# ZhangHH233/Retinal_OCT_Image_Segmentation_via_Deep_Learning

Measured on AMD Instinct MI355X. Metric: B-scans/sec (train fwd+bwd) at batch 32, 512x1024, higher is better.
Workload: dtype bf16; 1 GPU; SOTAS/Layers_Segment UNet(1,8,init_features=32) train step, 512x1024, batch 32/GPU (BASELINE configs[1]); global_batch=32, parallelism=dp1, hip_graph=False

## Files before the change

### include/oct_hip.h

```cpp
#ifndef OCT_HIP_H
#define OCT_HIP_H

#include <stddef.h>
#include <stdint.h>

#ifdef __cplusplus
extern "C" {
#endif

#define OCT_VERSION 220

#define OCT_DT_BF16 0
#define OCT_DT_F32 1

#define OCT_OK 0
#define OCT_IMG_SHIFT_ALL 2
#define OCT_E_INVALID (-22)
#define OCT_E_LAUNCH (-5)
#define OCT_E_NODEVICE (-19)

#define OCT_XF_NONE 0
#define OCT_XF_AFFINE_RELU 1
#define OCT_XF_AFFINE 2

#define OCT_IN_PLAIN 0
#define OCT_IN_S2D 1
#define OCT_OUT_PLAIN 0
#define OCT_OUT_D2S 1

#define OCT_PACK_CONV_FPROP 0
#define OCT_PACK_CONV_DGRAD 1
#define OCT_PACK_DECONV_FPROP 2
#define OCT_PACK_DECONV_DGRAD 3
#define OCT_PACK_1X1_DGRAD 4
#define OCT_PACK_1X1_FPROP 5
#define OCT_PACK_CONV3D_FPROP 6
#define OCT_PACK_CONV3D_DGRAD 7
#define OCT_PACK_DECONV3D_FPROP 8
#define OCT_PACK_DECONV3D_DGRAD 9

const char* oct_version_string(void);
int oct_version(void);
int oct_get_last_error(char* buf, size_t len);
int oct_device_count(void);

typedef struct OctConvDesc {
  int dtype;
  int n, h, w;
  int c0, c1;
  int cout;
  int taps;
  int xform0, xform1;
  int in_mode, out_mode;
  int split;
  int want_stats;
  int kh, kw;
  int depth;
  int out_img_mul, out_img_add;
} OctConvDesc;

typedef struct OctConvArgs {
  const void* x0; const void* x1;
  const float* scale0; const float* shift0;
  const float* scale1; const float* shift1;
  const void* wpacked;
  const float* bias;
  void* y0; void* y1;
  float* stat_partials;
} OctConvArgs;

int oct_conv_stat_blocks(const OctConvDesc* d);
size_t oct_packed_weight_elems(int rows, int taps, int kch);
int oct_pack_weights(int mode, int dtype, const float* w, void* wpacked, int cout, int cin, void* stream);
int oct_pack_weights_kk(int mode, int dtype, const float* w, void* wpacked, int cout, int cin, int kh, int kw,
                        void* stream);
int oct_pack_weights3d(int mode, int dtype, const float* w, void* wpacked, int cout, int cin, int kdi, void* stream);
#define OCT_PACK_BATCH_MAX 96
typedef struct OctPackJob {
  int mode, cout, cin, reserved;
  const float* w;
  void* wpacked;
} OctPackJob;
int oct_pack_weights_batch(int dtype, int count, const OctPackJob* jobs, void* stream);
int oct_conv_forward(const OctConvDesc* d, const OctConvArgs* a, void* stream);

typedef struct OctWgradDesc {
  int dtype;
  int n, h, w;
  int c0, c1;
  int cout;
  int taps;
  int xform0, xform1;
  int dy_mode;
  int kh, kw;
  int depth;
  int in_img_shift;
  int dy_img_mul, dy_img_add;
  int partials;
} OctWgradDesc;
typedef struct OctWgradArgs {
  const void* x0; const void* x1;
  const float* scale0; const float* shift0;
  const float* scale1; const float* shift1;
  const void* dy;
  float* dwp;
  float* dbias;
  const void* dy_y; const float* dy_coef; const float* dy_scale; const float* dy_shift;
  float* dbias_partials;
} OctWgradArgs;
int oct_conv_wgrad(const OctWgradDesc* d, const OctWgradArgs* a, void* stream);
int oct_conv_wgrad_partials(const OctWgradDesc* d);
int oct_reduce_bias_partials(const float* part, int nparts, int rows, int channels, float* dbias, int accumulate,
                             void* stream);
int oct_conv_wgrad_fused_apply_ok(const OctWgradDesc* d);
int oct_conv_wgrad_all_depth_taps_ok(const OctWgradDesc* d);
typedef struct OctConvBwdFusedArgs {
  const void* x;
  const float* scale; const float* shift;
  const float* mean; const float* invstd;
  const void* dy;
  const void* wpacked;
  void* dx;
  float* dwp;
  float* partials;
} OctConvBwdFusedArgs;
int oct_conv_backward_fused_ok(const OctWgradDesc* d);
int oct_conv_backward_fused_blocks(const OctWgradDesc* d);
int oct_conv_backward_fused(const OctWgradDesc* d, const OctConvBwdFusedArgs* a, void* stream);
int oct_unpack_wgrad(int mode, const float* dwp, float* grad, int cout, int cin, int accumulate, void* stream);
int oct_unpack_wgrad_kk(const float* dwp, float* grad, int cout, int cin, int kh, int kw, int accumulate, void* stream);
int oct_unpack_wgrad3d(int mode, const float* dwp, float* grad, int cout, int cin, int kdi, int accumulate, void* stream);
typedef struct OctUnpackJob {
  int mode, cout, cin, accumulate;
  int nparts, reserved;
  const float* dwp;
  float* grad;
} OctUnpackJob;
int oct_unpack_wgrad_batch(int count, const OctUnpackJob* jobs, void* stream);

int oct_bn_finalize(const float* partials, int nblocks, int c, double count,
                    const float* gamma, const float* beta, float eps, float momentum,
                    float* running_mean, float* running_var,
                    float* mean, float* invstd, float* scale, float* shift, const float* conv_bias,
                    void* stream);
int oct_bn_eval_coeffs(int c, const float* gamma, const float* beta, const float* running_mean,
                       const float* running_var, float eps, float* scale, float* shift,
                       const float* conv_bias, void* stream);

int oct_bn_relu_pool_fwd(int dtype, const void* y, const float* scale, const float* shift,
                         void* pooled, int n, int h, int w, int c, void* stream);
int oct_bn_relu_fwd(int dtype, const void* y, const float* scale, const float* shift,
                    void* out, size_t npix, int c, void* stream);

int oct_dact_bn_reduce(int dtype, const void* da, const void* dpool, const void* y,
                       const float* scale, const float* shift, const float* mean,
                       const float* invstd, void* g, float* partials, int n, int h, int w, int c,
                       void* stream);
int oct_dact_bn_reduce_blocks(int n, int h, int w, int c, int has_pool);
int oct_bn_bwd_apply_pool_ok(int dtype, int n, int h, int w, int c);
int oct_bn_bwd_apply_pool(int dtype, const void* da, const void* dpool, const void* y, const float* scale,
                          const float* shift, const float* coef, void* dy, int n, int h, int w, int c, void* stream);
int oct_bn_bwd_finalize(const float* partials, int nblocks, int c, double count,
                        const float* gamma, const float* mean, const float* invstd,
                        float* dgamma, float* dbeta, float* coef , int accumulate,
                        void* stream);
int oct_bn_bwd_apply(int dtype, void* g, const void* y, const float* coef, const float* scale,
                     const float* shift, size_t npix, int c, void* stream);
int oct_bn_bwd_apply_to(int dtype, void* dst, const void* g, const void* y, const float* coef, const float* scale,
                        const float* shift, size_t npix, int c, void* stream);
int oct_rowdot_ok(int c, int k);
int oct_rowdot_blocks(size_t npix, int c);
int oct_rowdot_fwd(int dtype, const void* x, const float* w, void* y, float* stats, size_t npix, int c, int k, void* stream);
int oct_rowdot_bwd_data(int dtype, const void* dy, const float* w, void* dx, size_t npix, int c, int k, void* stream);
int oct_rowdot_bwd_weight(int dtype, const void* dy, const void* x, float* dw, float* partials, size_t npix, int c, int k,
                          int accumulate, void* stream);
int oct_rowdot_bwd_weight_bias(int dtype, const void* dy, const void* x, float* dw, float* dbias, float* partials, size_t npix, int c,
                               int k, int accumulate, void* stream);

int oct_channel_sum(int dtype, const void* x, float* out, size_t npix, int c, int accumulate,
                    void* stream);

typedef struct OctHeadDesc {
  int dtype;
  int n, h, w;
  int feat;
  int classes;
} OctHeadDesc;
#define OCT_MAX_CLASSES 16
#define OCT_HEAD_LOSS_SLOTS (2 + 3 * OCT_MAX_CLASSES)
int oct_head_blocks(const OctHeadDesc* d);
int oct_head_forward(const OctHeadDesc* d, const void* y, const float* scale, const float* shift,
                     const float* w , const float* b, const int64_t* target,
                     float* probs, int64_t* argmax, float* logits ,
                     double* loss_partials, void* stream);
int oct_head_loss_finalize(const OctHeadDesc* d, const double* loss_partials, int nblocks,
                           float w_ce, float w_dice, float dice_eps, float* loss_out,
                           float* dice_coef, void* stream);
int oct_head_dlogits(const OctHeadDesc* d, const void* y, const float* scale, const float* shift,
                     const float* w, const float* b, const int64_t* target, const float* dice_coef,
                     float w_ce, const float* dprobs, void* dlogits, void* stream);

int oct_head_backward_fused(const OctHeadDesc* d, const void* y, const float* scale, const float* shift,
                            const float* mean, const float* invstd, const float* w, const float* b,
                            const int64_t* target, const float* dice_coef, float w_ce,
                            const float* dprobs, void* dlogits, void* da, float* partials,
                            float* dbias, float* dweight, double* loss_partials, void* stream);

#define OCT_SEG_NHWC 0
#define OCT_SEG_NCHW 1
int oct_seg_loss_blocks(size_t npix, int classes);
int oct_seg_loss_forward(const OctHeadDesc* d, int layout, const void* logits, const int64_t* target,
                         int64_t* argmax, double* loss_partials, void* stream);
int oct_seg_loss_backward(const OctHeadDesc* d, int layout, const void* logits, const int64_t* target,
                          const float* dice_coef, float w_ce, const float* dloss, void* dlogits,
                          double* loss_partials, void* stream);

int oct_seg_loss_weight_sum(const OctHeadDesc* d, const int64_t* target, const float* class_weight,
                            const float* pixel_weight, int has_ignore, int64_t ignore_index,
                            double* partials, double* wsum, void* stream);
int oct_seg_loss_forward_weighted(const OctHeadDesc* d, int layout, const void* logits,
                                  const int64_t* target, const float* class_weight,
                                  const float* pixel_weight, int has_ignore, int64_t ignore_index,
                                  double* loss_partials, void* stream);
int oct_seg_loss_backward_weighted(const OctHeadDesc* d, int layout, const void* logits,
                                   const int64_t* target, const float* class_weight,
                                   const float* pixel_weight, int has_ignore, int64_t ignore_index,
                                   const double* wsum, const float* dice_coef, float w_ce,
                                   const float* dloss, void* dlogits, double* loss_partials,
                                   void* stream);
int oct_seg_loss_finalize_weighted(const OctHeadDesc* d, const double* loss_partials, int nblocks,
                                   float w_ce, float w_dice, float dice_eps, float* loss_out,
                                   float* dice_coef, double* wsum_out, void* stream);

int oct_bce_loss_weight_sum(const OctHeadDesc* d, const uint8_t* target, const float* pixel_weight,
                            int has_ignore, int ignore_value, double* partials, double* wsum,
                            void* stream);
int oct_bce_loss_forward(const OctHeadDesc* d, int layout, const void* logits, const uint8_t* target,
                         const float* pos_weight, const float* pixel_weight, int has_ignore,
                         int ignore_value, int want_dice, float tau, uint8_t* mask,
                         double* loss_partials, void* stream);
int oct_bce_loss_backward(const OctHeadDesc* d, int layout, const void* logits, const uint8_t* target,
                          const float* pos_weight, const float* pixel_weight, int has_ignore,
                          int ignore_value, const double* wsum, const float* dice_coef, float w_bce,
                          const float* dloss, void* dlogits, double* loss_partials, void* stream);

int oct_nchw_to_nhwc(int dtype, const float* x, void* out, int n, int c, int h, int w, void* stream);
int oct_nhwc_to_nchw(int dtype, const void* x, float* out, int n, int c, int h, int w, void* stream);
int oct_sgd_step(float* p, const float* g, float* buf, size_t n, float lr, float momentum,
                 float weight_decay, float grad_scale, int first, void* stream);

int oct_adam_step(float* p, const float* g, float* m, float* v, size_t n, float lr, float beta1,
                  float beta2, float eps, float weight_decay, int decoupled, float step_size,
                  float inv_sqrt_bc2, float grad_scale, const float* dev_scale,
                  const uint8_t* decay_mask, void* stream);
int oct_sgd_step_scaled(float* p, const float* g, float* buf, size_t n, float lr, float momentum,
                        float weight_decay, float grad_scale, int first, const float* dev_scale,
                        const uint8_t* decay_mask, void* stream);
int oct_grad_norm_blocks(size_t n);
int oct_grad_norm(const float* g, size_t n, float grad_scale, float max_norm, double* partials,
                  float* out, void* stream);

#define OCT_ACT_NONE 0
#define OCT_ACT_RELU 1
#define OCT_ACT_SIGMOID 2
int oct_affine_act_fwd(int dtype, const void* y, const float* scale, const float* shift,
                       const void* res, int act, void* out, size_t npix, int c, void* stream);
int oct_affine_res_act_fwd(int dtype, const void* y, const float* scale, const float* shift, const void* res,
                           const float* res_shift, int act, void* out, size_t npix, int c, void* stream);
int oct_act_bwd(int dtype, const void* dout, const void* out, int act, void* dz, size_t n, void* stream);
int oct_maxpool_fwd(int dtype, const void* a, void* out, int n, int h, int w, int c, int k, void* stream);
int oct_maxpool_bwd(int dtype, const void* a, const void* dout, void* da, int n, int h, int w, int c,
                    int k, void* stream);
int oct_bilinear_up_fwd(int dtype, const void* x, void* out, int n, int h, int w, int c, int factor,
                        void* stream);
int oct_bilinear_up_bwd(int dtype, const void* dout, void* dx, int n, int h, int w, int c, int factor,
                        void* stream);
int oct_bilinear_resize_fwd(int dtype, const void* x, void* out, int n, int h, int w, int c, int ho, int wo,
                            void* stream);
int oct_bilinear_resize_bwd(int dtype, const void* dout, void* dx, int n, int h, int w, int c, int ho, int wo,
                            void* stream);
int oct_depth_to_space(int dtype, const void* in, const float* bias, void* out, int n, int h, int w,
                       int cout, int s, void* stream);
int oct_space_to_depth(int dtype, const void* in, void* out, int n, int h, int w, int cout, int s,
                       void* stream);
int oct_gate_fwd(int dtype, const void* x, const void* p, void* out, size_t npix, int c, void* stream);
int oct_gate_bwd(int dtype, const void* dout, const void* x, const void* p, void* dx, void* dp,
                 size_t npix, int c, void* stream);

int oct_affine_prelu_fwd(int dtype, const void* y, const float* scale, const float* shift, const float* alpha,
                         void* out, size_t npix, int c, void* stream);
int oct_affine_prelu_bwd(int dtype, const void* dout, const void* y, const float* scale, const float* shift,
                         const float* alpha, void* dz, float* dalpha, size_t npix, int c, void* stream);
int oct_prelu_bn_fused_ok(int dtype, int c);
int oct_dact_bn_reduce_prelu(int dtype, const void* da, const void* y, const float* scale, const float* shift, const float* alpha,
                             const float* mean, const float* invstd, float* partials, float* dalpha, int n, int h, int w, int c,
                             void* stream);
int oct_bn_bwd_apply_prelu_to(int dtype, void* dst, const void* da, const void* y, const float* coef, const float* scale,
                              const float* shift, const float* alpha, size_t npix, int c, void* stream);
int oct_maxpool_idx_fwd(int dtype, const void* a, void* out, int64_t* idx, int n, int h, int w, int c, int k, void* stream);
int oct_index_scatter(int dtype, const void* v, const int64_t* idx, void* out, int n, size_t npool, size_t plane, int c,
                      void* stream);
int oct_index_gather(int dtype, const void* x, const int64_t* idx, void* v, int n, size_t npool, size_t plane, int c,
                     void* stream);
int oct_maxpool_code_fwd(int dtype, const void* a, void* out, unsigned char* code, int n, int h, int w, int c, int k, void* stream);
int oct_window_scatter(int dtype, const void* v, const unsigned char* code, void* out, int n, int hp, int wp, int c, int k, void* stream);
int oct_window_gather(int dtype, const void* x, const unsigned char* code, void* v, int n, int hp, int wp, int c, int k, void* stream);

int oct_depth_pool_fwd(int dtype, const void* p2, void* out, size_t nslab, size_t m, void* stream);
int oct_depth_pool_bwd(int dtype, const void* p2, const void* dout, void* dp2, size_t nslab, size_t m, void* stream);

int oct_confusion_counts(const void* y_true, const void* y_pred, int elem, size_t n,
                         int64_t* out_i ,
                         double* out_f , void* stream);

int oct_class_confusion_counts(const void* y_true, const void* y_pred, int elem, size_t n, int classes,
                               int64_t* out , uint64_t* scratch ,
                               void* stream);

int oct_sqdiff_sum(const void* y_true, const void* y_pred, int elem, size_t n, double* out, void* stream);
int oct_column_absdiff_sum(const void* y_true, const void* y_pred, int elem, int unsigned_wrap, size_t rows,
                           size_t cols, double* out, void* stream);

#define OCT_EVAL_PRED_U8 0
#define OCT_EVAL_PRED_I64 1
#define OCT_EVAL_PRED_NHWC_BF16 2
#define OCT_EVAL_PRED_NHWC_F32 3
#define OCT_EVAL_PRED_NCHW_F32 4
#define OCT_EVAL_STATE_EXTRA 4
typedef struct {
  int images, h, w, classes;
  int target_elem;
  int pred_kind;
  int has_ignore;
  int64_t ignore_index;
} OctSegEvalDesc;
int oct_seg_eval_update(const OctSegEvalDesc* d, const void* target, const void* pred, int64_t* state, void* stream);

#ifdef __cplusplus
}
#endif
#endif
```

### retinal_oct_image_segmentation_via_deep_learning_amd/_lib.py

```python
from __future__ import annotations

import ctypes as C
import os
import subprocess
import threading

PKG_DIR = os.path.dirname(os.path.abspath(__file__))
LIB_PATH = os.environ.get("OCT_HIP_LIB") or os.path.join(PKG_DIR, "liboct_hip.so")
CSRC_DIR = os.path.join(PKG_DIR, "csrc")

DT_BF16, DT_F32 = 0, 1
XF_NONE, XF_AFFINE_RELU, XF_AFFINE = 0, 1, 2
IN_PLAIN, IN_S2D = 0, 1
IMG_SHIFT_ALL = 2
ACT_NONE, ACT_RELU, ACT_SIGMOID = 0, 1, 2
ACT_PRELU = 3
OUT_PLAIN, OUT_D2S = 0, 1
PACK_CONV_FPROP, PACK_CONV_DGRAD, PACK_DECONV_FPROP, PACK_DECONV_DGRAD, PACK_1X1_DGRAD, PACK_1X1_FPROP = range(6)
PACK_CONV3D_FPROP, PACK_CONV3D_DGRAD, PACK_DECONV3D_FPROP, PACK_DECONV3D_DGRAD = 6, 7, 8, 9
MAX_CLASSES = 16
HEAD_LOSS_SLOTS = 2 + 3 * MAX_CLASSES
SEG_NHWC, SEG_NCHW = 0, 1

c_void_p, c_int, c_size_t, c_float, c_double = C.c_void_p, C.c_int, C.c_size_t, C.c_float, C.c_double


class PackJob(C.Structure):
    _fields_ = [("mode", c_int), ("cout", c_int), ("cin", c_int), ("reserved", c_int), ("w", c_void_p),
                ("wpacked", c_void_p)]


class UnpackJob(C.Structure):
    _fields_ = [("mode", c_int), ("cout", c_int), ("cin", c_int), ("accumulate", c_int), ("nparts", c_int),
                ("reserved", c_int), ("dwp", c_void_p), ("grad", c_void_p)]


PACK_BATCH_MAX = 96


class ConvDesc(C.Structure):
    _fields_ = [(k, c_int) for k in (
        "dtype", "n", "h", "w", "c0", "c1", "cout", "taps", "xform0", "xform1", "in_mode", "out_mode",
        "split", "want_stats", "kh", "kw", "depth", "out_img_mul", "out_img_add")]


class ConvArgs(C.Structure):
    _fields_ = [(k, c_void_p) for k in (
        "x0", "x1", "scale0", "shift0", "scale1", "shift1", "wpacked", "bias", "y0", "y1", "stat_partials")]


class WgradDesc(C.Structure):
    _fields_ = [(k, c_int) for k in (
        "dtype", "n", "h", "w", "c0", "c1", "cout", "taps", "xform0", "xform1", "dy_mode", "kh", "kw", "depth",
        "in_img_shift", "dy_img_mul", "dy_img_add", "partials")]


class WgradArgs(C.Structure):
    _fields_ = [(k, c_void_p) for k in ("x0", "x1", "scale0", "shift0", "scale1", "shift1", "dy", "dwp", "dbias",
                                                "dy_y", "dy_coef", "dy_scale", "dy_shift", "dbias_partials")]


class ConvBwdFusedArgs(C.Structure):
    _fields_ = [(k, c_void_p) for k in ("x", "scale", "shift", "mean", "invstd", "dy", "wpacked", "dx", "dwp", "partials")]


class HeadDesc(C.Structure):
    _fields_ = [(k, c_int) for k in ("dtype", "n", "h", "w", "feat", "classes")]


class SegEvalDesc(C.Structure):
    _fields_ = [(k, c_int) for k in ("images", "h", "w", "classes", "target_elem", "pred_kind", "has_ignore")] + \
               [("ignore_index", C.c_int64)]


EVAL_PRED_U8, EVAL_PRED_I64, EVAL_PRED_NHWC_BF16, EVAL_PRED_NHWC_F32, EVAL_PRED_NCHW_F32 = range(5)
EVAL_STATE_EXTRA = 4


SIGNATURES = {
    "oct_version_string": (C.c_char_p, []),
    "oct_version": (c_int, []),
    "oct_get_last_error": (c_int, [C.c_char_p, c_size_t]),
    "oct_device_count": (c_int, []),
    "oct_conv_stat_blocks": (c_int, [C.POINTER(ConvDesc)]),
    "oct_packed_weight_elems": (c_size_t, [c_int, c_int, c_int]),
    "oct_pack_weights": (c_int, [c_int, c_int, c_void_p, c_void_p, c_int, c_int, c_void_p]),
    "oct_pack_weights3d": (c_int, [c_int, c_int, c_void_p, c_void_p, c_int, c_int, c_int, c_void_p]),
    "oct_unpack_wgrad3d": (c_int, [c_int, c_void_p, c_void_p, c_int, c_int, c_int, c_int, c_void_p]),
    "oct_depth_pool_fwd": (c_int, [c_int, c_void_p, c_void_p, c_size_t, c_size_t, c_void_p]),
    "oct_depth_pool_bwd": (c_int, [c_int, c_void_p, c_void_p, c_void_p, c_size_t, c_size_t, c_void_p]),
    "oct_pack_weights_kk": (c_int, [c_int, c_int, c_void_p, c_void_p, c_int, c_int, c_int, c_int, c_void_p]),
    "oct_unpack_wgrad_kk": (c_int, [c_void_p, c_void_p, c_int, c_int, c_int, c_int, c_int, c_void_p]),
    "oct_affine_prelu_fwd": (c_int, [c_int, c_void_p, c_void_p, c_void_p, c_void_p, c_void_p, c_size_t, c_int, c_void_p]),
    "oct_affine_prelu_bwd": (c_int, [c_int, c_void_p, c_void_p, c_void_p, c_void_p, c_void_p, c_void_p, c_void_p, c_size_t,
                                     c_int, c_void_p]),
    "oct_maxpool_idx_fwd": (c_int, [c_int, c_void_p, c_void_p, c_void_p, c_int, c_int, c_int, c_int, c_int, c_void_p]),
    "oct_index_scatter": (c_int, [c_int, c_void_p, c_void_p, c_void_p, c_int, c_size_t, c_size_t, c_int, c_void_p]),
    "oct_index_gather": (c_int, [c_int, c_void_p, c_void_p, c_void_p, c_int, c_size_t, c_size_t, c_int, c_void_p]),
    "oct_prelu_bn_fused_ok": (c_int, [c_int, c_int]),
    "oct_dact_bn_reduce_prelu": (c_int, [c_int, c_void_p, c_void_p, c_void_p, c_void_p, c_void_p, c_void_p, c_void_p, c_void_p, c_void_p,
                                         c_int, c_int, c_int, c_int, c_void_p]),
    "oct_bn_bwd_apply_prelu_to": (c_int, [c_int, c_void_p, c_void_p, c_void_p, c_void_p, c_void_p, c_void_p, c_void_p, c_size_t, c_int,
                                          c_void_p]),
    "oct_maxpool_code_fwd": (c_int, [c_int, c_void_p, c_void_p, c_void_p, c_int, c_int, c_int, c_int, c_int, c_void_p]),
    "oct_window_scatter": (c_int, [c_int, c_void_p, c_void_p, c_void_p, c_int, c_int, c_int, c_int, c_int, c_void_p]),
    "oct_window_gather": (c_int, [c_int, c_void_p, c_void_p, c_void_p, c_int, c_int, c_int, c_int, c_int, c_void_p]),
    "oct_pack_weights_batch": (c_int, [c_int, c_int, C.POINTER(PackJob), c_void_p]),
    "oct_conv_forward": (c_int, [C.POINTER(ConvDesc), C.POINTER(ConvArgs), c_void_p]),
    "oct_conv_wgrad": (c_int, [C.POINTER(WgradDesc), C.POINTER(WgradArgs), c_void_p]),
    "oct_conv_wgrad_fused_apply_ok": (c_int, [C.POINTER(WgradDesc)]),
    "oct_conv_wgrad_all_depth_taps_ok": (c_int, [C.POINTER(WgradDesc)]),
    "oct_conv_backward_fused_ok": (c_int, [C.POINTER(WgradDesc)]),
    "oct_conv_backward_fused_blocks": (c_int, [C.POINTER(WgradDesc)]),
    "oct_conv_backward_fused": (c_int, [C.POINTER(WgradDesc), C.POINTER(ConvBwdFusedArgs), c_void_p]),
    "oct_conv_wgrad_partials": (c_int, [C.POINTER(WgradDesc)]),
    "oct_reduce_bias_partials": (c_int, [c_void_p, c_int, c_int, c_int, c_void_p, c_int, c_void_p]),
    "oct_unpack_wgrad": (c_int, [c_int, c_void_p, c_void_p, c_int, c_int, c_int, c_void_p]),
    "oct_unpack_wgrad_batch": (c_int, [c_int, C.POINTER(UnpackJob), c_void_p]),
    "oct_bn_finalize": (c_int, [c_void_p, c_int, c_int, c_double, c_void_p, c_void_p, c_float, c_float,
                                c_void_p, c_void_p, c_void_p, c_void_p, c_void_p, c_void_p, c_void_p, c_void_p]),
    "oct_bn_eval_coeffs": (c_int, [c_int, c_void_p, c_void_p, c_void_p, c_void_p, c_float, c_void_p, c_void_p,
                                   c_void_p, c_void_p]),
    "oct_bn_relu_pool_fwd": (c_int, [c_int, c_void_p, c_void_p, c_void_p, c_void_p, c_int, c_int, c_int, c_int,
                                     c_void_p]),
    "oct_bn_relu_fwd": (c_int, [c_int, c_void_p, c_void_p, c_void_p, c_void_p, c_size_t, c_int, c_void_p]),
    "oct_dact_bn_reduce": (c_int, [c_int, c_void_p, c_void_p, c_void_p, c_void_p, c_void_p, c_void_p, c_void_p,
                                   c_void_p, c_void_p, c_int, c_int, c_int, c_int, c_void_p]),
    "oct_dact_bn_reduce_blocks": (c_int, [c_int, c_int, c_int, c_int, c_int]),
    "oct_bn_bwd_apply_pool_ok": (c_int, [c_int, c_int, c_int, c_int, c_int]),
    "oct_bn_bwd_apply_pool": (c_int, [c_int, c_void_p, c_void_p, c_void_p, c_void_p, c_void_p, c_void_p, c_void_p,
                                      c_int, c_int, c_int, c_int, c_void_p]),
    "oct_bn_bwd_finalize": (c_int, [c_void_p, c_int, c_int, c_double, c_void_p, c_void_p, c_void_p, c_void_p,
                                    c_void_p, c_void_p, c_int, c_void_p]),
    "oct_bn_bwd_apply": (c_int, [c_int, c_void_p, c_void_p, c_void_p, c_void_p, c_void_p, c_size_t, c_int,
                                 c_void_p]),
    "oct_bn_bwd_apply_to": (c_int, [c_int, c_void_p, c_void_p, c_void_p, c_void_p, c_void_p, c_void_p, c_size_t, c_int,
                                    c_void_p]),
    "oct_channel_sum": (c_int, [c_int, c_void_p, c_void_p, c_size_t, c_int, c_int, c_void_p]),
    "oct_rowdot_ok": (c_int, [c_int, c_int]),
    "oct_rowdot_blocks": (c_int, [c_size_t, c_int]),
    "oct_rowdot_fwd": (c_int, [c_int, c_void_p, c_void_p, c_void_p, c_void_p, c_size_t, c_int, c_int, c_void_p]),
    "oct_rowdot_bwd_data": (c_int, [c_int, c_void_p, c_void_p, c_void_p, c_size_t, c_int, c_int, c_void_p]),
    "oct_rowdot_bwd_weight": (c_int, [c_int, c_void_p, c_void_p, c_void_p, c_void_p, c_size_t, c_int, c_int, c_int, c_void_p]),
    "oct_rowdot_bwd_weight_bias": (c_int, [c_int, c_void_p, c_void_p, c_void_p, c_void_p, c_void_p, c_size_t, c_int, c_int, c_int,
                                           c_void_p]),
    "oct_head_blocks": (c_int, [C.POINTER(HeadDesc)]),
    "oct_head_forward": (c_int, [C.POINTER(HeadDesc), c_void_p, c_void_p, c_void_p, c_void_p, c_void_p, c_void_p,
                                 c_void_p, c_void_p, c_void_p, c_void_p, c_void_p]),
    "oct_head_loss_finalize": (c_int, [C.POINTER(HeadDesc), c_void_p, c_int, c_float, c_float, c_float, c_void_p,
                                       c_void_p, c_void_p]),
    "oct_head_dlogits": (c_int, [C.POINTER(HeadDesc), c_void_p, c_void_p, c_void_p, c_void_p, c_void_p, c_void_p,
                                 c_void_p, c_float, c_void_p, c_void_p, c_void_p]),
    "oct_head_backward_fused": (c_int, [C.POINTER(HeadDesc), c_void_p, c_void_p, c_void_p, c_void_p, c_void_p, c_void_p,
                                        c_void_p, c_void_p, c_void_p, c_float, c_void_p, c_void_p, c_void_p, c_void_p,
                                        c_void_p, c_void_p, c_void_p, c_void_p]),
    "oct_seg_loss_blocks": (c_int, [c_size_t, c_int]),
    "oct_seg_loss_forward": (c_int, [C.POINTER(HeadDesc), c_int, c_void_p, c_void_p, c_void_p, c_void_p, c_void_p]),
    "oct_seg_loss_backward": (c_int, [C.POINTER(HeadDesc), c_int, c_void_p, c_void_p, c_void_p, c_float, c_void_p, c_void_p,
                                      c_void_p, c_void_p]),
    "oct_seg_loss_weight_sum": (c_int, [C.POINTER(HeadDesc), c_void_p, c_void_p, c_void_p, c_int, C.c_int64, c_void_p, c_void_p,
                                        c_void_p]),
    "oct_seg_loss_forward_weighted": (c_int, [C.POINTER(HeadDesc), c_int, c_void_p, c_void_p, c_void_p, c_void_p, c_int,
                                              C.c_int64, c_void_p, c_void_p]),
    "oct_seg_loss_backward_weighted": (c_int, [C.POINTER(HeadDesc), c_int, c_void_p, c_void_p, c_void_p, c_void_p, c_int,
                                               C.c_int64, c_void_p, c_void_p, c_float, c_void_p, c_void_p, c_void_p, c_void_p]),
    "oct_seg_loss_finalize_weighted": (c_int, [C.POINTER(HeadDesc), c_void_p, c_int, c_float, c_float, c_float, c_void_p,
                                               c_void_p, c_void_p, c_void_p]),
    "oct_bce_loss_weight_sum": (c_int, [C.POINTER(HeadDesc), c_void_p, c_void_p, c_int, c_int, c_void_p, c_void_p, c_void_p]),
    "oct_bce_loss_forward": (c_int, [C.POINTER(HeadDesc), c_int, c_void_p, c_void_p, c_void_p, c_void_p, c_int, c_int, c_int,
                                     c_float, c_void_p, c_void_p, c_void_p]),
    "oct_bce_loss_backward": (c_int, [C.POINTER(HeadDesc), c_int, c_void_p, c_void_p, c_void_p, c_void_p, c_int, c_int,
                                      c_void_p, c_void_p, c_float, c_void_p, c_void_p, c_void_p, c_void_p]),
    "oct_nchw_to_nhwc": (c_int, [c_int, c_void_p, c_void_p, c_int, c_int, c_int, c_int, c_void_p]),
    "oct_nhwc_to_nchw": (c_int, [c_int, c_void_p, c_void_p, c_int, c_int, c_int, c_int, c_void_p]),
    "oct_sgd_step": (c_int, [c_void_p, c_void_p, c_void_p, c_size_t, c_float, c_float, c_float, c_float, c_int,
                             c_void_p]),
    "oct_adam_step": (c_int, [c_void_p, c_void_p, c_void_p, c_void_p, c_size_t, c_float, c_float, c_float, c_float, c_float,
                              c_int, c_float, c_float, c_float, c_void_p, c_void_p, c_void_p]),
    "oct_sgd_step_scaled": (c_int, [c_void_p, c_void_p, c_void_p, c_size_t, c_float, c_float, c_float, c_float, c_int,
                                    c_void_p, c_void_p, c_void_p]),
    "oct_grad_norm_blocks": (c_int, [c_size_t]),
    "oct_grad_norm": (c_int, [c_void_p, c_size_t, c_float, c_float, c_void_p, c_void_p, c_void_p]),
    "oct_affine_act_fwd": (c_int, [c_int, c_void_p, c_void_p, c_void_p, c_void_p, c_int, c_void_p, c_size_t, c_int,
                                   c_void_p]),
    "oct_affine_res_act_fwd": (c_int, [c_int, c_void_p, c_void_p, c_void_p, c_void_p, c_void_p, c_int, c_void_p, c_size_t,
                                       c_int, c_void_p]),
    "oct_act_bwd": (c_int, [c_int, c_void_p, c_void_p, c_int, c_void_p, c_size_t, c_void_p]),
    "oct_maxpool_fwd": (c_int, [c_int, c_void_p, c_void_p, c_int, c_int, c_int, c_int, c_int, c_void_p]),
    "oct_maxpool_bwd": (c_int, [c_int, c_void_p, c_void_p, c_void_p, c_int, c_int, c_int, c_int, c_int, c_void_p]),
    "oct_bilinear_up_fwd": (c_int, [c_int, c_void_p, c_void_p, c_int, c_int, c_int, c_int, c_int, c_void_p]),
    "oct_bilinear_up_bwd": (c_int, [c_int, c_void_p, c_void_p, c_int, c_int, c_int, c_int, c_int, c_void_p]),
    "oct_bilinear_resize_fwd": (c_int, [c_int, c_void_p, c_void_p, c_int, c_int, c_int, c_int, c_int, c_int, c_void_p]),
    "oct_bilinear_resize_bwd": (c_int, [c_int, c_void_p, c_void_p, c_int, c_int, c_int, c_int, c_int, c_int, c_void_p]),
    "oct_depth_to_space": (c_int, [c_int, c_void_p, c_void_p, c_void_p, c_int, c_int, c_int, c_int, c_int, c_void_p]),
    "oct_space_to_depth": (c_int, [c_int, c_void_p, c_void_p, c_int, c_int, c_int, c_int, c_int, c_void_p]),
    "oct_gate_fwd": (c_int, [c_int, c_void_p, c_void_p, c_void_p, c_size_t, c_int, c_void_p]),
    "oct_gate_bwd": (c_int, [c_int, c_void_p, c_void_p, c_void_p, c_void_p, c_void_p, c_size_t, c_int, c_void_p]),
    "oct_confusion_counts": (c_int, [c_void_p, c_void_p, c_int, c_size_t, c_void_p, c_void_p, c_void_p]),
    "oct_class_confusion_counts": (c_int, [c_void_p, c_void_p, c_int, c_size_t, c_int, c_void_p, c_void_p, c_void_p]),
    "oct_sqdiff_sum": (c_int, [c_void_p, c_void_p, c_int, c_size_t, c_void_p, c_void_p]),
    "oct_column_absdiff_sum": (c_int, [c_void_p, c_void_p, c_int, c_int, c_size_t, c_size_t, c_void_p, c_void_p]),
    "oct_seg_eval_update": (c_int, [C.POINTER(SegEvalDesc), c_void_p, c_void_p, c_void_p, c_void_p]),
}

_lib = None
_lock = threading.Lock()
param_generation = [0]


class OctError(RuntimeError):
    pass


def build(verbose: bool = False) -> str:
    cmd = ["make", "-C", CSRC_DIR, "-j8"]
    res = subprocess.run(cmd, capture_output=True, text=True)
    if verbose or res.returncode != 0:
        print(res.stdout[-4000:])
        print(res.stderr[-4000:])
    if res.returncode != 0:
        raise OctError("building liboct_hip.so failed (see output above)")
    return LIB_PATH


def lib():
    global _lib
    if _lib is not None:
        return _lib
    with _lock:
        if _lib is None:
            if not os.path.exists(LIB_PATH):
                raise OctError(
                    f"{LIB_PATH} is missing: the HIP extension has not been built "
                    "(run `python __graft_entry__.py` or `make -C .../csrc`). There is no CPU fallback.")
            handle = C.CDLL(LIB_PATH)
            for name, (res, args) in SIGNATURES.items():
                fn = getattr(handle, name)
                fn.restype = res
                fn.argtypes = args
            _lib = handle
    return _lib


def last_error() -> str:
    buf = C.create_string_buffer(512)
    lib().oct_get_last_error(buf, 512)
    return buf.value.decode("utf-8", "replace")


def check(rc: int, what: str = "") -> None:
    if rc != 0:
        raise OctError(f"{what or 'liboct_hip'} failed with code {rc}: {last_error()}")


def ptr(t) -> int | None:
    return None if t is None else t.data_ptr()
```

### retinal_oct_image_segmentation_via_deep_learning_amd/csrc/head.hip

```cpp
#include "common.h"

#include <stdlib.h>

#define HEAD_THREADS 256
int oct_head_backward_mfma(const OctHeadDesc* d, const void* y, const float* scale, const float* shift, const float* mean,
                           const float* invstd, const float* w, const float* b, const int64_t* target,
                           const float* dice_coef, float w_ce, void* da, float* partials, float* dbias, float* dweight,
                           double* loss_partials, int grid, void* stream);
#define HEAD_MAX_FEAT 128

struct HeadParams {
  const void* y; const float* scale; const float* shift; const float* w; const float* b;
  const int64_t* target; float* probs; int64_t* argmax; float* logits; double* loss_partials;
  const float* dice_coef; const float* dprobs; void* dlogits; float w_ce;
  int n, h, wd, feat, classes;
};

template <typename T, int CMAX>
__device__ __forceinline__ void head_logits(const HeadParams& p, size_t pix, const float* sw, const float* sb,
                                            const float* ssc, const float* ssh, float (&l)[CMAX]) {
  const T* y = reinterpret_cast<const T*>(p.y) + pix * p.feat;
#pragma unroll
  for (int c = 0; c < CMAX; ++c) l[c] = (c < p.classes) ? sb[c] : 0.f;
  if ((p.feat & 7) == 0) {
    for (int f0 = 0; f0 < p.feat; f0 += 8) {
      float a[8];
      load_vec<T, 8>(y + f0, a);
#pragma unroll
      for (int j = 0; j < 8; ++j) a[j] = fmaxf(fmaf(a[j], ssc[f0 + j], ssh[f0 + j]), 0.f);
#pragma unroll
      for (int c = 0; c < CMAX; ++c)
        if (c < p.classes) {
#pragma unroll
          for (int j = 0; j < 8; ++j) l[c] = fmaf(sw[c * p.feat + f0 + j], a[j], l[c]);
        }
    }
  } else {
    for (int f = 0; f < p.feat; ++f) {
      const float a = fmaxf(fmaf(to_f32(y[f]), ssc[f], ssh[f]), 0.f);
#pragma unroll
      for (int c = 0; c < CMAX; ++c)
        if (c < p.classes) l[c] = fmaf(sw[c * p.feat + f], a, l[c]);
    }
  }
}

template <int CMAX>
__device__ __forceinline__ void softmax_c(int classes, const float (&l)[CMAX], float (&pr)[CMAX], float& m, float& lse) {
  m = l[0];
#pragma unroll
  for (int c = 1; c < CMAX; ++c)
    if (c < classes) m = fmaxf(m, l[c]);
  float s = 0.f;
#pragma unroll
  for (int c = 0; c < CMAX; ++c) {
    pr[c] = (c < classes) ? expf(l[c] - m) : 0.f;
    s += pr[c];
  }
  const float inv = 1.f / s;
#pragma unroll
  for (int c = 0; c < CMAX; ++c) pr[c] *= inv;
  lse = logf(s);
}

__device__ __forceinline__ void head_load_consts(const HeadParams& p, float* sw, float* sb, float* ssc, float* ssh) {
  for (int i = threadIdx.x; i < p.classes * p.feat; i += blockDim.x) sw[i] = p.w[i];
  for (int i = threadIdx.x; i < p.classes; i += blockDim.x) sb[i] = p.b[i];
  for (int i = threadIdx.x; i < p.feat; i += blockDim.x) { ssc[i] = p.scale[i]; ssh[i] = p.shift[i]; }
  __syncthreads();
}

template <typename T, int CMAX>
__global__ void __launch_bounds__(HEAD_THREADS) head_fwd_kernel(const HeadParams p) {
  __shared__ float sw[OCT_MAX_CLASSES * HEAD_MAX_FEAT];
  __shared__ float sb[OCT_MAX_CLASSES], ssc[HEAD_MAX_FEAT], ssh[HEAD_MAX_FEAT];
  __shared__ double red[HEAD_THREADS / 64][OCT_HEAD_LOSS_SLOTS];
  head_load_consts(p, sw, sb, ssc, ssh);
  const size_t hw = (size_t)p.h * p.wd, npix = (size_t)p.n * hw;
  float ce = 0.f, si[CMAX], sp[CMAX], sy[CMAX];
#pragma unroll
  for (int c = 0; c < CMAX; ++c) { si[c] = 0.f; sp[c] = 0.f; sy[c] = 0.f; }
  for (size_t pix = (size_t)blockIdx.x * blockDim.x + threadIdx.x; pix < npix; pix += (size_t)gridDim.x * blockDim.x) {
    float l[CMAX], pr[CMAX], m, lse;
    head_logits<T, CMAX>(p, pix, sw, sb, ssc, ssh, l);
    softmax_c<CMAX>(p.classes, l, pr, m, lse);
    const size_t img = pix / hw, off = pix - img * hw;
    if (p.logits) {
#pragma unroll
      for (int c = 0; c < CMAX; ++c)
        if (c < p.classes) p.logits[(img * p.classes + c) * hw + off] = l[c];
    }
    if (p.probs) {
#pragma unroll
      for (int c = 0; c < CMAX; ++c)
        if (c < p.classes) p.probs[(img * p.classes + c) * hw + off] = pr[c];
    }
    if (p.argmax) {
      int best = 0; float bv = pr[0];
#pragma unroll
      for (int c = 1; c < CMAX; ++c)
        if (c < p.classes && pr[c] > bv) { bv = pr[c]; best = c; }
      p.argmax[pix] = best;
    }
    if (p.target) {
      const int t = (int)p.target[pix];
#pragma unroll
      for (int c = 0; c < CMAX; ++c) {
        const bool hit = (c == t);
        if (hit) ce -= (l[c] - m - lse);
        si[c] += hit ? pr[c] : 0.f;
        sp[c] += pr[c];
        sy[c] += hit ? 1.f : 0.f;
      }
      if ((unsigned)t >= (unsigned)p.classes) ce = __builtin_nanf("");
    }
  }
  if (p.loss_partials) {
    const int wave = threadIdx.x >> 6, lane = threadIdx.x & 63;
    double v = wave_sum((double)ce);
    if (lane == 0) { red[wave][0] = v; red[wave][1] = 0.0; }
#pragma unroll
    for (int c = 0; c < CMAX; ++c) {
      const double a = wave_sum((double)si[c]), b = wave_sum((double)sp[c]), d = wave_sum((double)sy[c]);
      if (lane == 0) {
        red[wave][2 + c] = a; red[wave][2 + OCT_MAX_CLASSES + c] = b; red[wave][2 + 2 * OCT_MAX_CLASSES + c] = d;
      }
    }
    if (lane == 0)
      for (int c = CMAX; c < OCT_MAX_CLASSES; ++c) {
        red[wave][2 + c] = 0.0; red[wave][2 + OCT_MAX_CLASSES + c] = 0.0; red[wave][2 + 2 * OCT_MAX_CLASSES + c] = 0.0;
      }
    __syncthreads();
    for (int i = threadIdx.x; i < OCT_HEAD_LOSS_SLOTS; i += blockDim.x) {
      double s = 0.0;
      for (int wv = 0; wv < HEAD_THREADS / 64; ++wv) s += red[wv][i];
      p.loss_partials[(size_t)blockIdx.x * OCT_HEAD_LOSS_SLOTS + i] = s;
    }
  }
}

__global__ void __launch_bounds__(1024) head_loss_finalize_kernel(const double* __restrict__ partials, int nblocks, int classes, double npix,
                                          float w_ce, float w_dice, float eps, float* loss_out, float* dice_coef) {
  __shared__ double tot[OCT_HEAD_LOSS_SLOTS];
  __shared__ double part[16][64];
  {
    const int slot = threadIdx.x & 63, seg = threadIdx.x >> 6;
    double sv[8] = {0.0, 0.0, 0.0, 0.0, 0.0, 0.0, 0.0, 0.0};
    if (slot < OCT_HEAD_LOSS_SLOTS) {
      int b = seg;
      for (; b + 7 * 16 < nblocks; b += 8 * 16) {
#pragma unroll
        for (int u = 0; u < 8; ++u) sv[u] += partials[(size_t)(b + 16 * u) * OCT_HEAD_LOSS_SLOTS + slot];
      }
      for (; b < nblocks; b += 16) sv[0] += partials[(size_t)b * OCT_HEAD_LOSS_SLOTS + slot];
    }
    part[seg][slot] = ((sv[0] + sv[1]) + (sv[2] + sv[3])) + ((sv[4] + sv[5]) + (sv[6] + sv[7]));
    __syncthreads();
    if (threadIdx.x < OCT_HEAD_LOSS_SLOTS) {
      double a = 0.0;
      for (int k = 0; k < 16; ++k) a += part[k][slot];
      tot[threadIdx.x] = a;
    }
  }
  __syncthreads();
  if (threadIdx.x == 0) {
    const double ce = tot[0] / npix;
    double dsum = 0.0;
    for (int c = 0; c < classes; ++c) {
      const double I = tot[2 + c], P = tot[2 + OCT_MAX_CLASSES + c], Y = tot[2 + 2 * OCT_MAX_CLASSES + c];
      const double den = P + Y + (double)eps, num = 2.0 * I + (double)eps;
      dsum += num / den;
      dice_coef[c] = (float)(-(double)w_dice / classes * 2.0 / den);
      dice_coef[OCT_MAX_CLASSES + c] = (float)((double)w_dice / classes * num / (den * den));
    }
    const double dice = 1.0 - dsum / classes;
    loss_out[0] = (float)((double)w_ce * ce + (double)w_dice * dice);
    loss_out[1] = (float)ce;
    loss_out[2] = (float)dice;
  }
}

template <typename T, int CMAX>
__global__ void __launch_bounds__(HEAD_THREADS) head_dlogits_kernel(const HeadParams p) {
  __shared__ float sw[OCT_MAX_CLASSES * HEAD_MAX_FEAT];
  __shared__ float sb[OCT_MAX_CLASSES], ssc[HEAD_MAX_FEAT], ssh[HEAD_MAX_FEAT];
  __shared__ float sdc[2 * OCT_MAX_CLASSES];
  if (p.dice_coef) for (int i = threadIdx.x; i < 2 * OCT_MAX_CLASSES; i += blockDim.x) sdc[i] = p.dice_coef[i];
  head_load_consts(p, sw, sb, ssc, ssh);
  const size_t hw = (size_t)p.h * p.wd, npix = (size_t)p.n * hw;
  const float inv_n = 1.f / (float)npix;
  T* out = reinterpret_cast<T*>(p.dlogits);
  for (size_t pix = (size_t)blockIdx.x * blockDim.x + threadIdx.x; pix < npix; pix += (size_t)gridDim.x * blockDim.x) {
    float l[CMAX], pr[CMAX], dp[CMAX], m, lse;
    head_logits<T, CMAX>(p, pix, sw, sb, ssc, ssh, l);
    softmax_c<CMAX>(p.classes, l, pr, m, lse);
    float dl[CMAX];
    if (p.dprobs) {
      const size_t img = pix / hw, off = pix - img * hw;
      float dot = 0.f;
#pragma unroll
      for (int c = 0; c < CMAX; ++c) {
        dp[c] = (c < p.classes) ? p.dprobs[(img * p.classes + c) * hw + off] : 0.f;
        dot = fmaf(pr[c], dp[c], dot);
      }
#pragma unroll
      for (int c = 0; c < CMAX; ++c) dl[c] = pr[c] * (dp[c] - dot);
    } else {
      const int t = (int)p.target[pix];
      float dot = 0.f;
#pragma unroll
      for (int c = 0; c < CMAX; ++c) {
        dp[c] = 0.f;
        if (p.dice_coef && c < p.classes) dp[c] = (c == t ? sdc[c] : 0.f) + sdc[OCT_MAX_CLASSES + c];
        dot = fmaf(pr[c], dp[c], dot);
      }
#pragma unroll
      for (int c = 0; c < CMAX; ++c)
        dl[c] = p.w_ce * (pr[c] - (c == t ? 1.f : 0.f)) * inv_n + pr[c] * (dp[c] - dot);
    }
#pragma unroll
    for (int c = 0; c < CMAX; ++c)
      if (c < p.classes) out[pix * p.classes + c] = from_f32<T>(dl[c]);
  }
}

__device__ __forceinline__ float quad_xor1(float v) {
  return __builtin_bit_cast(float, __builtin_amdgcn_update_dpp(0, __builtin_bit_cast(int, v), 0xB1, 0xF, 0xF, true));
}
__device__ __forceinline__ float quad_xor2(float v) {
  return __builtin_bit_cast(float, __builtin_amdgcn_update_dpp(0, __builtin_bit_cast(int, v), 0x4E, 0xF, 0xF, true));
}

template <typename T, int CMAX, bool DW>
__global__ void __launch_bounds__(HEAD_THREADS) head_bwd_fused_kernel(const HeadParams p, const float* __restrict__ mean,
                                                                       const float* __restrict__ invstd, T* __restrict__ da_out,
                                                                       float* __restrict__ partials, float* __restrict__ dbias,
                                                                       float* __restrict__ dweight, double* __restrict__ loss_partials) {
  constexpr int F = 32, G = 4, PPB = HEAD_THREADS / G;
  __shared__ float red[HEAD_THREADS / 64][2 * F + OCT_MAX_CLASSES];
  __shared__ double redce[HEAD_THREADS / 64];
  float ce = 0.f;
  __shared__ float sdw[DW ? CMAX * F : 1];
  const int g = threadIdx.x & 3, slot = threadIdx.x >> 2;
  const int wave = threadIdx.x >> 6, lane = threadIdx.x & 63;
  float w[CMAX][8], bias[CMAX], sc[8], sh[8], mu[8], is[8], dcA[CMAX], dcB[CMAX];
#pragma unroll
  for (int c = 0; c < CMAX; ++c) {
    bias[c] = c < p.classes ? p.b[c] : 0.f;
    dcA[c] = (p.dice_coef && c < p.classes) ? p.dice_coef[c] : 0.f;
    dcB[c] = (p.dice_coef && c < p.classes) ? p.dice_coef[OCT_MAX_CLASSES + c] : 0.f;
#pragma unroll
    for (int j = 0; j < 8; ++j) w[c][j] = c < p.classes ? p.w[c * F + g * 8 + j] : 0.f;
  }
#pragma unroll
  for (int j = 0; j < 8; ++j) {
    sc[j] = p.scale[g * 8 + j]; sh[j] = p.shift[g * 8 + j]; mu[j] = mean[g * 8 + j]; is[j] = invstd[g * 8 + j];
  }
  if (DW) {
    for (int i = threadIdx.x; i < CMAX * F; i += HEAD_THREADS) sdw[i] = 0.f;
    __syncthreads();
  }
  const size_t hw = (size_t)p.h * p.wd, npix = (size_t)p.n * hw;
  const float inv_n = 1.f / (float)npix;
  float s1[8], s2[8], sdb[CMAX], dwa[DW ? CMAX : 1][8];
#pragma unroll
  for (int j = 0; j < 8; ++j) { s1[j] = 0.f; s2[j] = 0.f; }
#pragma unroll
  for (int c = 0; c < CMAX; ++c) {
    sdb[c] = 0.f;
    if (DW) {
#pragma unroll
      for (int j = 0; j < 8; ++j) dwa[c][j] = 0.f;
    }
  }
  T* dl_out = reinterpret_cast<T*>(p.dlogits);
  const T* ybase = reinterpret_cast<const T*>(p.y);
  const size_t stride = (size_t)gridDim.x * PPB;
  size_t pix = (size_t)blockIdx.x * PPB + slot;
  float yn[8];
  int tn = 0;
  {
    const size_t q = pix < npix ? pix : 0;
    load_vec<T, 8>(ybase + q * F + g * 8, yn);
    if (p.target) tn = (int)p.target[q];
  }
  for (; pix < npix; pix += stride) {
    float yv[8], z[8], a[8], l[CMAX], pr[CMAX], dl[CMAX], m, lse;
    const int t = tn;
#pragma unroll
    for (int j = 0; j < 8; ++j) yv[j] = yn[j];
    {
      const size_t q = pix + stride < npix ? pix + stride : pix;
      load_vec<T, 8>(ybase + q * F + g * 8, yn);
      if (p.target) tn = (int)p.target[q];
    }
#pragma unroll
    for (int j = 0; j < 8; ++j) { z[j] = fmaf(yv[j], sc[j], sh[j]); a[j] = fmaxf(z[j], 0.f); }
#pragma unroll
    for (int c = 0; c < CMAX; ++c) {
      float s = 0.f;
#pragma unroll
      for (int j = 0; j < 8; ++j) s = fmaf(w[c][j], a[j], s);
      s += quad_xor1(s);
      s += quad_xor2(s);
      l[c] = s + bias[c];
    }
    softmax_c<CMAX>(p.classes, l, pr, m, lse);
    if (p.dprobs) {
      const size_t img = pix / hw, off = pix - img * hw;
      float dp[CMAX], dot = 0.f;
#pragma unroll
      for (int c = 0; c < CMAX; ++c) {
        dp[c] = (c < p.classes) ? p.dprobs[(img * p.classes + c) * hw + off] : 0.f;
        dot = fmaf(pr[c], dp[c], dot);
      }
#pragma unroll
      for (int c = 0; c < CMAX; ++c) dl[c] = pr[c] * (dp[c] - dot);
    } else {
      float dp[CMAX], dot = 0.f;
#pragma unroll
      for (int c = 0; c < CMAX; ++c) {
        dp[c] = (c == t ? dcA[c] : 0.f) + dcB[c];
        dot = fmaf(pr[c], dp[c], dot);
      }
#pragma unroll
      for (int c = 0; c < CMAX; ++c) dl[c] = p.w_ce * (pr[c] - (c == t ? 1.f : 0.f)) * inv_n + pr[c] * (dp[c] - dot);
      if (loss_partials && g == 0) {
        float lt = 0.f;
#pragma unroll
        for (int c = 0; c < CMAX; ++c) lt = (c == t) ? l[c] : lt;
        ce -= lt - m - lse;
        if ((unsigned)t >= (unsigned)p.classes) ce = __builtin_nanf("");
      }
    }
#pragma unroll
    for (int c = 0; c < CMAX; ++c) {
      dl[c] = (c < p.classes) ? to_f32(from_f32<T>(dl[c])) : 0.f;
      if (g == 0) sdb[c] += dl[c];
    }
    if (dl_out && g == 0) {
#pragma unroll
      for (int c = 0; c < CMAX; ++c)
        if (c < p.classes) dl_out[pix * p.classes + c] = from_f32<T>(dl[c]);
    }
    float dav[8];
#pragma unroll
    for (int j = 0; j < 8; ++j) {
      float d = 0.f;
#pragma unroll
      for (int c = 0; c < CMAX; ++c) d = fmaf(w[c][j], dl[c], d);
      dav[j] = d;
      const float dr = to_f32(from_f32<T>(d));
      const float gm = z[j] > 0.f ? dr : 0.f;
      s1[j] += gm;
      s2[j] = fmaf(gm, (yv[j] - mu[j]) * is[j], s2[j]);
    }
    store_vec<T, 8>(da_out + pix * F + g * 8, dav);
    if (DW) {
#pragma unroll
      for (int j = 0; j < 8; ++j) {
        const float ar = to_f32(from_f32<T>(a[j]));
#pragma unroll
        for (int c = 0; c < CMAX; ++c) dwa[c][j] = fmaf(dl[c], ar, dwa[c][j]);
      }
    }
  }
#pragma unroll
  for (int j = 0; j < 8; ++j) {
    float a = s1[j], b = s2[j];
#pragma unroll
    for (int o = 32; o >= G; o >>= 1) { a += __shfl_xor(a, o); b += __shfl_xor(b, o); }
    if (lane < G) { red[wave][g * 8 + j] = a; red[wave][F + g * 8 + j] = b; }
  }
#pragma unroll
  for (int c = 0; c < CMAX; ++c) {
    const float a = wave_sum(sdb[c]);
    if (lane == 0) red[wave][2 * F + c] = a;
  }
  if (DW) {
#pragma unroll
    for (int c = 0; c < CMAX; ++c)
#pragma unroll
      for (int j = 0; j < 8; ++j) {
        float v = dwa[c][j];
#pragma unroll
        for (int o = 32; o >= G; o >>= 1) v += __shfl_xor(v, o);
        if (lane < G) atomicAdd(&sdw[c * F + g * 8 + j], v);
      }
  }
  __syncthreads();
  for (int i = threadIdx.x; i < 2 * F + CMAX; i += blockDim.x) {
    float s = 0.f;
    for (int wv = 0; wv < HEAD_THREADS / 64; ++wv) s += red[wv][i];
    if (i < 2 * F) partials[(size_t)blockIdx.x * 2 * F + i] = s;
    else if (i - 2 * F < p.classes) atomicAdd(&dbias[i - 2 * F], s);
  }
  if (DW) {
    for (int i = threadIdx.x; i < p.classes * F; i += blockDim.x) atomicAdd(&dweight[i], sdw[i]);
  }
  if (loss_partials) {
    const double v = wave_sum((double)ce);
    if (lane == 0) redce[wave] = v;
    __syncthreads();
    for (int i = threadIdx.x; i < OCT_HEAD_LOSS_SLOTS; i += blockDim.x) {
      double s = 0.0;
      if (i == 0) for (int wv = 0; wv < HEAD_THREADS / 64; ++wv) s += redce[wv];
      loss_partials[(size_t)blockIdx.x * OCT_HEAD_LOSS_SLOTS + i] = s;
    }
  }
}

static int head_grid(const OctHeadDesc* d) {
  const size_t npix = (size_t)d->n * d->h * d->w;
  size_t b = (npix + HEAD_THREADS - 1) / HEAD_THREADS;
  if (b > 2048) b = 2048;
  return (int)b;
}
extern "C" int oct_head_blocks(const OctHeadDesc* d) { return d ? head_grid(d) : 0; }

static int head_check(const OctHeadDesc* d, const char* who) {
  OCT_CHECK(d, "%s: null descriptor", who);
  OCT_CHECK(d->dtype == OCT_DT_BF16 || d->dtype == OCT_DT_F32, "%s: bad dtype %d", who, d->dtype);
  OCT_CHECK(d->n > 0 && d->h > 0 && d->w > 0, "%s: bad shape", who);
  OCT_CHECK(d->feat > 0 && d->feat <= HEAD_MAX_FEAT, "%s: feat %d not in [1,%d]", who, d->feat, HEAD_MAX_FEAT);
  OCT_CHECK(d->classes > 0 && d->classes <= OCT_MAX_CLASSES, "%s: classes %d not in [1,%d]", who, d->classes, OCT_MAX_CLASSES);
  return OCT_OK;
}

#define HEAD_DISPATCH(KERNEL, d, grid, s, p)                                                           \
  do {                                                                                                 \
    const int cm = (d)->classes <= 2 ? 2 : (d)->classes <= 4 ? 4 : (d)->classes <= 8 ? 8 : 16;         \
    if ((d)->dtype == OCT_DT_BF16) {                                                                   \
      if (cm == 2) hipLaunchKernelGGL((KERNEL<bf16_t, 2>), dim3(grid), dim3(HEAD_THREADS), 0, s, p);   \
      else if (cm == 4) hipLaunchKernelGGL((KERNEL<bf16_t, 4>), dim3(grid), dim3(HEAD_THREADS), 0, s, p); \
      else if (cm == 8) hipLaunchKernelGGL((KERNEL<bf16_t, 8>), dim3(grid), dim3(HEAD_THREADS), 0, s, p); \
      else hipLaunchKernelGGL((KERNEL<bf16_t, 16>), dim3(grid), dim3(HEAD_THREADS), 0, s, p);          \
    } else {                                                                                           \
      if (cm == 2) hipLaunchKernelGGL((KERNEL<float, 2>), dim3(grid), dim3(HEAD_THREADS), 0, s, p);    \
      else if (cm == 4) hipLaunchKernelGGL((KERNEL<float, 4>), dim3(grid), dim3(HEAD_THREADS), 0, s, p); \
      else if (cm == 8) hipLaunchKernelGGL((KERNEL<float, 8>), dim3(grid), dim3(HEAD_THREADS), 0, s, p); \
      else hipLaunchKernelGGL((KERNEL<float, 16>), dim3(grid), dim3(HEAD_THREADS), 0, s, p);           \
    }                                                                                                  \
  } while (0)

extern "C" int oct_head_forward(const OctHeadDesc* d, const void* y, const float* scale, const float* shift,
                                const float* w, const float* b, const int64_t* target, float* probs,
                                int64_t* argmax, float* logits, double* loss_partials, void* stream) {
  int rc = head_check(d, "oct_head_forward");
  if (rc) return rc;
  OCT_CHECK(y && scale && shift && w && b, "oct_head_forward: null pointer");
  OCT_CHECK(!(loss_partials && !target), "oct_head_forward: loss partials need a target");
  HeadParams p = {};
  p.y = y; p.scale = scale; p.shift = shift; p.w = w; p.b = b; p.target = target; p.probs = probs;
  p.argmax = argmax; p.logits = logits; p.loss_partials = target ? loss_partials : nullptr;
  p.n = d->n; p.h = d->h; p.wd = d->w; p.feat = d->feat; p.classes = d->classes;
  if (!loss_partials) p.target = nullptr;
  const int grid = head_grid(d);
  hipStream_t s = as_stream(stream);
  HEAD_DISPATCH(head_fwd_kernel, d, grid, s, p);
  return oct_check_launch("head_fwd");
}

extern "C" int oct_head_loss_finalize(const OctHeadDesc* d, const double* loss_partials, int nblocks, float w_ce,
                                      float w_dice, float dice_eps, float* loss_out, float* dice_coef, void* stream) {
  int rc = head_check(d, "oct_head_loss_finalize");
  if (rc) return rc;
  OCT_CHECK(loss_partials && loss_out && dice_coef && nblocks > 0, "oct_head_loss_finalize: bad args");
  hipLaunchKernelGGL(head_loss_finalize_kernel, dim3(1), dim3(1024), 0, as_stream(stream), loss_partials, nblocks,
                     d->classes, (double)d->n * d->h * d->w, w_ce, w_dice, dice_eps, loss_out, dice_coef);
  return oct_check_launch("head_loss_finalize");
}

extern "C" int oct_head_dlogits(const OctHeadDesc* d, const void* y, const float* scale, const float* shift,
                                const float* w, const float* b, const int64_t* target, const float* dice_coef,
                                float w_ce, const float* dprobs, void* dlogits, void* stream) {
  int rc = head_check(d, "oct_head_dlogits");
  if (rc) return rc;
  OCT_CHECK(y && scale && shift && w && b && dlogits, "oct_head_dlogits: null pointer");
  OCT_CHECK(target || dprobs, "oct_head_dlogits: need a target or dprobs");
  HeadParams p = {};
  p.y = y; p.scale = scale; p.shift = shift; p.w = w; p.b = b; p.target = target; p.dice_coef = dice_coef;
  p.dprobs = dprobs; p.dlogits = dlogits; p.w_ce = w_ce;
  p.n = d->n; p.h = d->h; p.wd = d->w; p.feat = d->feat; p.classes = d->classes;
  const int grid = head_grid(d);
  hipStream_t s = as_stream(stream);
  HEAD_DISPATCH(head_dlogits_kernel, d, grid, s, p);
  return oct_check_launch("head_dlogits");
}

extern "C" int oct_head_backward_fused(const OctHeadDesc* d, const void* y, const float* scale, const float* shift,
                                       const float* mean, const float* invstd, const float* w, const float* b,
                                       const int64_t* target, const float* dice_coef, float w_ce, const float* dprobs,
                                       void* dlogits, void* da, float* partials, float* dbias, float* dweight,
                                       double* loss_partials, void* stream) {
  int rc = head_check(d, "oct_head_backward_fused");
  if (rc) return rc;
  OCT_CHECK(d->feat == 32, "oct_head_backward_fused: only feat == 32 is fused (got %d); use oct_head_dlogits", d->feat);
  OCT_CHECK(y && scale && shift && mean && invstd && w && b && da && partials && dbias, "oct_head_backward_fused: null pointer");
  OCT_CHECK(target || dprobs, "oct_head_backward_fused: need a target or dprobs");
  HeadParams p = {};
  p.y = y; p.scale = scale; p.shift = shift; p.w = w; p.b = b; p.target = target; p.dice_coef = dice_coef;
  p.dprobs = dprobs; p.dlogits = dlogits; p.w_ce = w_ce;
  p.n = d->n; p.h = d->h; p.wd = d->w; p.feat = d->feat; p.classes = d->classes;
  OCT_CHECK(!dweight || d->classes <= 8, "oct_head_backward_fused: the fused weight gradient needs classes <= 8 (got %d)", d->classes);
  OCT_CHECK(dlogits || dweight, "oct_head_backward_fused: without dlogits the weight gradient must be fused (dweight)");
  OCT_CHECK(!loss_partials || target, "oct_head_backward_fused: loss partials need a target");
  {
    static int mfma_on = -1;
    if (mfma_on < 0) { const char* e = getenv("OCT_HEAD_MFMA"); mfma_on = (e && e[0] == '0') ? 0 : 1; }
    if (mfma_on && d->dtype == OCT_DT_BF16 && d->classes <= 8 && target && !dprobs && dweight && !dlogits)
      return oct_head_backward_mfma(d, y, scale, shift, mean, invstd, w, b, target, dice_coef, w_ce, da, partials, dbias,
                                    dweight, loss_partials, head_grid(d), stream);
  }
  const int grid = head_grid(d);
  hipStream_t s = as_stream(stream);
  const int cm = d->classes <= 2 ? 2 : d->classes <= 4 ? 4 : d->classes <= 8 ? 8 : 16;
#define LAUNCH(T, C, W) hipLaunchKernelGGL((head_bwd_fused_kernel<T, C, W>), dim3(grid), dim3(HEAD_THREADS), 0, s, p, mean, \
                                           invstd, (T*)da, partials, dbias, dweight, loss_partials)
#define BYCLS(T, W)                                                                                   \
  do {                                                                                                \
    if (cm == 2) LAUNCH(T, 2, W); else if (cm == 4) LAUNCH(T, 4, W); else LAUNCH(T, 8, W);            \
  } while (0)
  if (cm == 16) { if (d->dtype == OCT_DT_BF16) LAUNCH(bf16_t, 16, false); else LAUNCH(float, 16, false); }
  else if (d->dtype == OCT_DT_BF16) { if (dweight) BYCLS(bf16_t, true); else BYCLS(bf16_t, false); }
  else { if (dweight) BYCLS(float, true); else BYCLS(float, false); }
#undef BYCLS
#undef LAUNCH
  return oct_check_launch("head_bwd_fused");
}
```

### retinal_oct_image_segmentation_via_deep_learning_amd/csrc/head_mfma.hip

```cpp
#include "common.h"

#define HM_THREADS 256

struct HeadMfmaParams {
  const bf16_t* y; const float* scale; const float* shift; const float* mean; const float* invstd;
  const float* w; const float* b; const int64_t* target; const float* dice_coef;
  bf16_t* da; float* partials; float* dbias; float* dweight; double* loss_partials;
  float w_ce; int classes; unsigned npix;
};

typedef unsigned int hm_u32x4 __attribute__((ext_vector_type(4)));
typedef short hm_s16x4 __attribute__((ext_vector_type(4)));

__device__ __forceinline__ bf16x8 hm_tr_frag(const unsigned char* base_lo) {
  typedef __attribute__((address_space(3))) hm_s16x4 lds_s16x4;
  const hm_s16x4 a = __builtin_amdgcn_ds_read_tr16_b64_v4i16((lds_s16x4*)(base_lo));
  const hm_s16x4 b = __builtin_amdgcn_ds_read_tr16_b64_v4i16((lds_s16x4*)(base_lo + 4 * 64));
  typedef short s16x8 __attribute__((ext_vector_type(8)));
  const s16x8 v = {a[0], a[1], a[2], a[3], b[0], b[1], b[2], b[3]};
  return __builtin_bit_cast(bf16x8, v);
}

__device__ __forceinline__ unsigned hm_pack(float a, float b) {
  typedef __bf16 bf16x2 __attribute__((ext_vector_type(2)));
  bf16x2 v;
  v[0] = (bf16_t)a;
  v[1] = (bf16_t)b;
  return __builtin_bit_cast(unsigned, v);
}
__device__ __forceinline__ float hm_lo(unsigned u) { return __uint_as_float(u << 16); }
__device__ __forceinline__ float hm_hi(unsigned u) { return __uint_as_float(u & 0xffff0000u); }
__device__ __forceinline__ float hm_other(float v) { return __shfl_xor(v, 32); }
__device__ __forceinline__ unsigned hm_other(unsigned v) { return (unsigned)__shfl_xor((int)v, 32); }

__global__ void __launch_bounds__(HM_THREADS, 2) head_bwd_mfma_kernel(const HeadMfmaParams p) {
  typedef Mma<bf16_t> M;
  typedef M::Frag Frag;
  constexpr int F = 32;
  __shared__ float red[HM_THREADS / 64][2 * F + 8];
  __shared__ float sdw[8 * F];
  __shared__ __attribute__((aligned(16))) unsigned char tiles[HM_THREADS / 64][2][32 * 64];
  __shared__ float sdc[2 * OCT_MAX_CLASSES];
  __shared__ double redce[HM_THREADS / 64];
  const int tid = threadIdx.x, lane = tid & 63, wave = tid >> 6;
  const int r = lane & 31, hh = lane >> 5;
  const int ncls = p.classes;
  for (int i = tid; i < 8 * F; i += HM_THREADS) sdw[i] = 0.f;
  for (int i = tid; i < (int)sizeof(tiles) / 4; i += HM_THREADS) reinterpret_cast<unsigned*>(&tiles[0][0][0])[i] = 0u;
  if (p.dice_coef) for (int i = tid; i < 2 * OCT_MAX_CLASSES; i += HM_THREADS) sdc[i] = p.dice_coef[i];
  __syncthreads();

  Frag wl_hi[2], wl_lo[2];
#pragma unroll
  for (int s = 0; s < 2; ++s)
#pragma unroll
    for (int j = 0; j < 8; ++j) {
      const float v = r < ncls ? p.w[r * F + 16 * s + 8 * hh + j] : 0.f;
      const bf16_t h = (bf16_t)v;
      wl_hi[s][j] = h;
      wl_lo[s][j] = (bf16_t)(v - (float)h);
    }
  Frag wt_hi, wt_lo;
#pragma unroll
  for (int j = 0; j < 8; ++j) {
    const int c = 8 * hh + j;
    const float v = c < ncls ? p.w[c * F + r] : 0.f;
    const bf16_t h = (bf16_t)v;
    wt_hi[j] = h;
    wt_lo[j] = (bf16_t)(v - (float)h);
  }
  float sc[16], sh[16];
#pragma unroll
  for (int q = 0; q < 2; ++q)
#pragma unroll
    for (int j = 0; j < 8; ++j) { sc[8 * q + j] = p.scale[16 * q + 8 * hh + j]; sh[8 * q + j] = p.shift[16 * q + 8 * hh + j]; }
  float bias4[4];
#pragma unroll
  for (int i = 0; i < 4; ++i) bias4[i] = (4 * hh + i) < ncls ? p.b[4 * hh + i] : 0.f;

  float s1[16], s2[16], sdb[4], ce = 0.f;
  f32x16 accw;
#pragma unroll
  for (int k = 0; k < 16; ++k) { s1[k] = 0.f; s2[k] = 0.f; accw[k] = 0.f; }
#pragma unroll
  for (int i = 0; i < 4; ++i) sdb[i] = 0.f;
  unsigned char* const a_tile = &tiles[wave][0][0];
  unsigned char* const d_tile = &tiles[wave][1][0];
  const int g4 = lane >> 4, li = lane & 15;
  const int tr_off = (8 * (g4 >> 1) + (li >> 2)) * 64 + (16 * (g4 & 1) + 4 * (li & 3)) * 2;
  const float inv_n = 1.f / (float)p.npix;

  const unsigned ngroups = (p.npix + 31) / 32;
  const unsigned gstride = gridDim.x * (HM_THREADS / 64);
  unsigned grp = blockIdx.x * (HM_THREADS / 64) + wave;
  hm_u32x4 yn0, yn1;
  int tn;
  {
    const unsigned px = grp < ngroups ? min(grp * 32 + r, p.npix - 1) : 0u;
    yn0 = *reinterpret_cast<const hm_u32x4*>(p.y + (size_t)px * F + 8 * hh);
    yn1 = *reinterpret_cast<const hm_u32x4*>(p.y + (size_t)px * F + 16 + 8 * hh);
    tn = (int)p.target[px];
  }
  for (; grp < ngroups; grp += gstride) {
    const unsigned pix = grp * 32 + r;
    const bool valid = pix < p.npix;
    const hm_u32x4 y0 = yn0, y1 = yn1;
    const int t = tn;
    {
      const unsigned g2 = grp + gstride < ngroups ? grp + gstride : grp;
      const unsigned px = min(g2 * 32 + r, p.npix - 1);
      yn0 = *reinterpret_cast<const hm_u32x4*>(p.y + (size_t)px * F + 8 * hh);
      yn1 = *reinterpret_cast<const hm_u32x4*>(p.y + (size_t)px * F + 16 + 8 * hh);
      tn = (int)p.target[px];
    }
    float yv[16], av[16];
    unsigned apk[8];
#pragma unroll
    for (int j = 0; j < 4; ++j) {
      yv[2 * j] = hm_lo(y0[j]); yv[2 * j + 1] = hm_hi(y0[j]);
      yv[8 + 2 * j] = hm_lo(y1[j]); yv[8 + 2 * j + 1] = hm_hi(y1[j]);
    }
    unsigned zmask = 0;
#pragma unroll
    for (int k = 0; k < 16; ++k) {
      const float z = fmaf(yv[k], sc[k], sh[k]);
      zmask |= z > 0.f ? (1u << k) : 0u;
      av[k] = fmaxf(z, 0.f);
    }
#pragma unroll
    for (int j = 0; j < 8; ++j) apk[j] = hm_pack(av[2 * j], av[2 * j + 1]);
    const hm_u32x4 a0 = {apk[0], apk[1], apk[2], apk[3]}, a1 = {apk[4], apk[5], apk[6], apk[7]};
    const Frag xa0 = __builtin_bit_cast(Frag, a0), xa1 = __builtin_bit_cast(Frag, a1);

    f32x16 acc;
#pragma unroll
    for (int i = 0; i < 16; ++i) acc[i] = 0.f;
    M::mma(acc, wl_hi[0], xa0); M::mma(acc, wl_lo[0], xa0);
    M::mma(acc, wl_hi[1], xa1); M::mma(acc, wl_lo[1], xa1);
    float l[4], pr[4], dl[4];
#pragma unroll
    for (int i = 0; i < 4; ++i) l[i] = (4 * hh + i) < ncls ? acc[i] + bias4[i] : -INFINITY;
    float m = fmaxf(fmaxf(l[0], l[1]), fmaxf(l[2], l[3]));
    m = fmaxf(m, hm_other(m));
    float s = 0.f;
#pragma unroll
    for (int i = 0; i < 4; ++i) { pr[i] = (4 * hh + i) < ncls ? expf(l[i] - m) : 0.f; s += pr[i]; }
    s += hm_other(s);
    const float inv = 1.f / s;
#pragma unroll
    for (int i = 0; i < 4; ++i) pr[i] *= inv;
#pragma unroll
    for (int i = 0; i < 4; ++i) dl[i] = p.w_ce * (pr[i] - ((4 * hh + i) == t ? 1.f : 0.f)) * inv_n;
    if (p.dice_coef) {
      float dp[4], dot = 0.f;
#pragma unroll
      for (int i = 0; i < 4; ++i) {
        const int c = 4 * hh + i;
        dp[i] = c < ncls ? (c == t ? sdc[c] : 0.f) + sdc[OCT_MAX_CLASSES + c] : 0.f;
        dot = fmaf(pr[i], dp[i], dot);
      }
      dot += hm_other(dot);
#pragma unroll
      for (int i = 0; i < 4; ++i) dl[i] = fmaf(pr[i], dp[i] - dot, dl[i]);
    }
    if (p.loss_partials) {
      float lt = 0.f;
      bool mine = false;
#pragma unroll
      for (int i = 0; i < 4; ++i)
        if ((4 * hh + i) == t) { lt = l[i]; mine = true; }
      if (mine && valid) ce -= lt - m - logf(s);
      if (valid && (unsigned)t >= (unsigned)ncls) ce = __builtin_nanf("");
    }
    unsigned dpk[2];
#pragma unroll
    for (int i = 0; i < 4; ++i) {
      dl[i] = (valid && (4 * hh + i) < ncls) ? (float)(bf16_t)dl[i] : 0.f;
      sdb[i] += dl[i];
    }
    dpk[0] = hm_pack(dl[0], dl[1]); dpk[1] = hm_pack(dl[2], dl[3]);
    const unsigned o0 = hm_other(dpk[0]), o1 = hm_other(dpk[1]);
    const hm_u32x4 dfr = {hh ? 0u : dpk[0], hh ? 0u : dpk[1], hh ? 0u : o0, hh ? 0u : o1};
    const Frag xd = __builtin_bit_cast(Frag, dfr);
    f32x16 acd;
#pragma unroll
    for (int i = 0; i < 16; ++i) acd[i] = 0.f;
    M::mma(acd, wt_hi, xd); M::mma(acd, wt_lo, xd);
    unsigned cpk[8];
#pragma unroll
    for (int g = 0; g < 4; ++g) {
      cpk[2 * g] = hm_pack(acd[4 * g], acd[4 * g + 1]);
      cpk[2 * g + 1] = hm_pack(acd[4 * g + 2], acd[4 * g + 3]);
    }
    const unsigned sA0 = hh ? cpk[0] : cpk[2], sA1 = hh ? cpk[1] : cpk[3];
    const unsigned sB0 = hh ? cpk[4] : cpk[6], sB1 = hh ? cpk[5] : cpk[7];
    const unsigned rA0 = hm_other(sA0), rA1 = hm_other(sA1), rB0 = hm_other(sB0), rB1 = hm_other(sB1);
    unsigned dq[8];
    if (hh == 0) {
      dq[0] = cpk[0]; dq[1] = cpk[1]; dq[2] = rA0; dq[3] = rA1;
      dq[4] = cpk[4]; dq[5] = cpk[5]; dq[6] = rB0; dq[7] = rB1;
    } else {
      dq[0] = rA0; dq[1] = rA1; dq[2] = cpk[2]; dq[3] = cpk[3];
      dq[4] = rB0; dq[5] = rB1; dq[6] = cpk[6]; dq[7] = cpk[7];
    }
    if (valid) {
      const hm_u32x4 o0v = {dq[0], dq[1], dq[2], dq[3]}, o1v = {dq[4], dq[5], dq[6], dq[7]};
      *reinterpret_cast<hm_u32x4*>(p.da + (size_t)pix * F + 8 * hh) = o0v;
      *reinterpret_cast<hm_u32x4*>(p.da + (size_t)pix * F + 16 + 8 * hh) = o1v;
    }
#pragma unroll
    for (int k = 0; k < 16; ++k) {
      const float d = (k & 1) ? hm_hi(dq[k >> 1]) : hm_lo(dq[k >> 1]);
      const float gm = (valid && ((zmask >> k) & 1u)) ? d : 0.f;
      s1[k] += gm;
      s2[k] = fmaf(gm, yv[k], s2[k]);
    }
    *reinterpret_cast<hm_u32x4*>(a_tile + r * 64 + 16 * hh) = a0;
    *reinterpret_cast<hm_u32x4*>(a_tile + r * 64 + 32 + 16 * hh) = a1;
    if (hh == 0) *reinterpret_cast<hm_u32x4*>(d_tile + r * 64) = dfr;
#pragma unroll
    for (int k16 = 0; k16 < 2; ++k16)
      M::mma(accw, hm_tr_frag(d_tile + k16 * 16 * 64 + tr_off), hm_tr_frag(a_tile + k16 * 16 * 64 + tr_off));
  }

#pragma unroll
  for (int k = 0; k < 16; ++k) {
    float a = s1[k], b = s2[k];
#pragma unroll
    for (int o = 16; o > 0; o >>= 1) { a += __shfl_xor(a, o); b += __shfl_xor(b, o); }
    if (r == 0) {
      const int f = 16 * (k >> 3) + 8 * hh + (k & 7);
      red[wave][f] = a; red[wave][F + f] = b;
    }
  }
#pragma unroll
  for (int i = 0; i < 4; ++i) {
    float a = sdb[i];
#pragma unroll
    for (int o = 16; o > 0; o >>= 1) a += __shfl_xor(a, o);
    if (r == 0) red[wave][2 * F + 4 * hh + i] = a;
  }
#pragma unroll
  for (int i = 0; i < 16; ++i) {
    const int c = (i & 3) + 8 * (i >> 2) + 4 * hh;
    if (c < ncls) atomicAdd(&sdw[c * F + r], accw[i]);
  }
  if (p.loss_partials) {
    const double v = wave_sum((double)ce);
    if (lane == 0) redce[wave] = v;
  }
  __syncthreads();
  for (int i = tid; i < 2 * F + 8; i += HM_THREADS) {
    float s = 0.f;
    for (int wv = 0; wv < HM_THREADS / 64; ++wv) s += red[wv][i];
    if (i < F) p.partials[(size_t)blockIdx.x * 2 * F + i] = s;
    else if (i < 2 * F) {
      float sg = 0.f;
      for (int wv = 0; wv < HM_THREADS / 64; ++wv) sg += red[wv][i - F];
      p.partials[(size_t)blockIdx.x * 2 * F + i] = (s - p.mean[i - F] * sg) * p.invstd[i - F];
    } else if (i - 2 * F < ncls) atomicAdd(&p.dbias[i - 2 * F], s);
  }
  for (int i = tid; i < ncls * F; i += HM_THREADS) atomicAdd(&p.dweight[i], sdw[i]);
  if (p.loss_partials) {
    for (int i = tid; i < OCT_HEAD_LOSS_SLOTS; i += HM_THREADS) {
      double s = 0.0;
      if (i == 0) for (int wv = 0; wv < HM_THREADS / 64; ++wv) s += redce[wv];
      p.loss_partials[(size_t)blockIdx.x * OCT_HEAD_LOSS_SLOTS + i] = s;
    }
  }
}

int oct_head_backward_mfma(const OctHeadDesc* d, const void* y, const float* scale, const float* shift, const float* mean,
                           const float* invstd, const float* w, const float* b, const int64_t* target,
                           const float* dice_coef, float w_ce, void* da, float* partials, float* dbias, float* dweight,
                           double* loss_partials, int grid, void* stream) {
  HeadMfmaParams p;
  p.y = (const bf16_t*)y; p.scale = scale; p.shift = shift; p.mean = mean; p.invstd = invstd; p.w = w; p.b = b;
  p.target = target; p.dice_coef = dice_coef; p.da = (bf16_t*)da; p.partials = partials; p.dbias = dbias;
  p.dweight = dweight; p.loss_partials = loss_partials; p.w_ce = w_ce; p.classes = d->classes;
  p.npix = (unsigned)((size_t)d->n * d->h * d->w);
  hipLaunchKernelGGL(head_bwd_mfma_kernel, dim3(grid), dim3(HM_THREADS), 0, as_stream(stream), p);
  return oct_check_launch("head_bwd_mfma");
}
```

### retinal_oct_image_segmentation_via_deep_learning_amd/engine.py

```python
from __future__ import annotations

import ctypes as C
import os
from dataclasses import dataclass, field

import torch

from . import _lib as L

BN_EPS = 1e-5
BN_MOMENTUM = 0.1

@dataclass
class ConvKeys:
    w: str
    bn: str
    b: str | None = None


@dataclass
class BlockSpec:
    name: str
    c1: ConvKeys
    c2: ConvKeys
    cout: int


@dataclass
class NetSpec:
    cin: int
    ncls: int
    enc: list
    ups: list
    dec: list
    head_w: str
    head_b: str
    dec_first: bool
    softmax_out: bool

    @property
    def divisor(self) -> int:
        return 1 << (len(self.enc) - 1)

    @property
    def head_feat(self) -> int:
        return self.dec[-1].cout


def ynet_unet_spec(cin: int, ncls: int, f: int) -> NetSpec:
    def blk(mod, pre, cout):
        return BlockSpec(pre, ConvKeys(f"{mod}.{pre}conv1.weight", f"{mod}.{pre}norm1"),
                         ConvKeys(f"{mod}.{pre}conv2.weight", f"{mod}.{pre}norm2"), cout)
    enc = [blk(f"encoder{i + 1}", f"enc{i + 1}", f << i) for i in range(4)] + [blk("bottleneck", "bottleneck", f * 16)]
    ups = [(f"upconv{k}.weight", f"upconv{k}.bias", f << (k - 1)) for k in (4, 3, 2, 1)]
    dec = [blk(f"decoder{k}", f"dec{k}", f << (k - 1)) for k in (4, 3, 2, 1)]
    return NetSpec(cin, ncls, enc, ups, dec, "conv.weight", "conv.bias", dec_first=True, softmax_out=True)


def bionet_unet_spec(cin: int, ncls: int) -> NetSpec:
    def blk(mod, cout):
        return BlockSpec(mod, ConvKeys(f"{mod}.0.weight", f"{mod}.1", f"{mod}.0.bias"),
                         ConvKeys(f"{mod}.3.weight", f"{mod}.4", f"{mod}.3.bias"), cout)
    enc = [blk("enc1", 64), blk("enc2", 128), blk("enc3", 256), blk("enc4", 512)]
    ups = [(f"up{k}.weight", f"up{k}.bias", c) for k, c in ((4, 256), (3, 128), (2, 64))]
    dec = [blk("dec4", 256), blk("dec3", 128), blk("dec2", 64)]
    return NetSpec(cin, ncls, enc, ups, dec, "final.weight", "final.bias", dec_first=False, softmax_out=False)


def _stream() -> int:
    return torch.cuda.current_stream().cuda_stream


@dataclass
class Src:
    x0: torch.Tensor
    c0: int
    bn0: "BNState | None" = None
    x1: torch.Tensor | None = None
    c1: int = 0
    bn1: "BNState | None" = None

    @property
    def channels(self) -> int:
        return self.c0 + self.c1


@dataclass
class BNState:
    scale: torch.Tensor
    shift: torch.Tensor
    mean: torch.Tensor | None = None
    invstd: torch.Tensor | None = None
    relu: bool = True
    frozen: bool = False


def _xf(bn) -> int:
    return L.XF_NONE if bn is None else (L.XF_AFFINE_RELU if bn.relu else L.XF_AFFINE)


@dataclass
class ConvRec:
    wkey: str
    gkey: str
    bkey: str
    cbkey: str | None
    src: Src
    y: torch.Tensor
    bn: BNState
    cout: int
    n: int
    h: int
    w: int


@dataclass
class Ctx:
    n: int = 0
    h: int = 0
    w: int = 0
    convs: dict = field(default_factory=dict)
    ups: dict = field(default_factory=dict)
    head_in: ConvRec | None = None
    target: torch.Tensor | None = None
    dice_coef: torch.Tensor | None = None
    loss: torch.Tensor | None = None
    loss_cfg: tuple = (1.0, 0.0, 1e-7)
    loss_partials: torch.Tensor | None = None


class UNetEngine:
    def __init__(self, in_channels: int, out_channels: int, features: int = 32, dtype: str = "bf16",
                 spec: NetSpec | None = None):
        if out_channels > L.MAX_CLASSES:
            raise L.OctError(f"out_channels={out_channels} exceeds the head kernel's limit {L.MAX_CLASSES}")
        self.spec = spec if spec is not None else ynet_unet_spec(in_channels, out_channels, features)
        self.cin, self.ncls, self.f = self.spec.cin, self.spec.ncls, self.spec.head_feat
        self.set_dtype(dtype)
        self._packed = {}
        self._arena, self._arena_on, self._arena_off, self._arena_short = None, False, 0, False
        self._unpack_jobs = []
        self._nbt = []
        self._frozen_bwd = False
        self.supports_frozen_bwd = True
        self._consts = {}
        self.rowdot_off = os.environ.get("OCT_ROWDOT", "1") == "0"
        self.deterministic = os.environ.get("OCT_DETERMINISTIC", "0") == "1"
        self.fused_bwd_off = False
        self.debug = None
        self.prof = None
        self.prof_labels = None

    def set_dtype(self, dtype: str) -> None:
        if dtype not in ("bf16", "f32"):
            raise ValueError("dtype must be 'bf16' or 'f32'")
        self.dtype = dtype
        self.dt = L.DT_BF16 if dtype == "bf16" else L.DT_F32
        self.tdt = torch.bfloat16 if dtype == "bf16" else torch.float32
        self._packed = {}
        self._pack_plan = {}

    def _prof_begin(self):
        if self.prof is None:
            return None
        ev = torch.cuda.Event(enable_timing=True)
        ev.record()
        return ev

    def _prof_end(self, ev, kind, label=None):
        if ev is not None:
            end = torch.cuda.Event(enable_timing=True)
            end.record()
            self.prof.append((kind, ev, end))
            if self.prof_labels is not None:
                self.prof_labels.append(label)

    def _const(self, value: float, n: int, dev):
        key = (float(value), int(n), str(dev))
        t = self._consts.get(key)
        if t is None:
            t = self._consts[key] = torch.full((n,), float(value), dtype=torch.float32, device=dev)
        return t

    def _act(self, n, h, w, c, dev):
        return torch.empty((n, h, w, c), dtype=self.tdt, device=dev)

    def _pack(self, key: str, wt: torch.Tensor, mode: int, cout: int, cin: int, kdi: int = 0) -> torch.Tensor:
        ver = (wt._version, L.param_generation[0])
        hit = self._packed.get((key, mode))
        if hit is not None and hit[0] == ver and hit[2] == wt.data_ptr():
            return hit[1]
        self._pack_plan[(key, mode)] = (cout, cin)
        rows, taps, kch = {
            L.PACK_CONV_FPROP: (cout, 9, cin), L.PACK_CONV_DGRAD: (cin, 9, cout),
            L.PACK_DECONV_FPROP: (4 * cout, 1, cin), L.PACK_DECONV_DGRAD: (cin, 1, 4 * cout),
            L.PACK_1X1_DGRAD: (cin, 1, cout), L.PACK_1X1_FPROP: (cout, 1, cin),
            L.PACK_CONV3D_FPROP: (cout, 9, 3 * cin), L.PACK_CONV3D_DGRAD: (cin, 9, 3 * cout),
            L.PACK_DECONV3D_FPROP: (4 * cout, 1, cin), L.PACK_DECONV3D_DGRAD: (cin, 1, 8 * cout)}[mode]
        elems = L.lib().oct_packed_weight_elems(rows, taps, kch)
        out = hit[1] if hit is not None else torch.empty(elems, dtype=self.tdt, device=wt.device)
        if mode >= L.PACK_CONV3D_FPROP:
            self._pack_plan.pop((key, mode), None)
            L.check(L.lib().oct_pack_weights3d(mode, self.dt, wt.data_ptr(), out.data_ptr(), cout, cin, kdi, _stream()),
                    "oct_pack_weights3d")
        else:
            L.check(L.lib().oct_pack_weights(mode, self.dt, wt.data_ptr(), out.data_ptr(), cout, cin, _stream()),
                    "oct_pack_weights")
        self._packed[(key, mode)] = (ver, out, wt.data_ptr())
        return out

    def _prepack(self, P: dict) -> None:
        jobs, news = [], []
        for (key, mode), (cout, cin) in self._pack_plan.items():
            wt = P.get(key) if isinstance(key, str) else None
            hit = self._packed.get((key, mode))
            if wt is None or hit is None or hit[2] != wt.data_ptr():
                continue
            ver = (wt._version, L.param_generation[0])
            if hit[0] != ver:
                jobs.append(L.PackJob(mode, cout, cin, 0, wt.data_ptr(), hit[1].data_ptr()))
                news.append(((key, mode), (ver, hit[1], hit[2])))
        if jobs:
            arr = (L.PackJob * len(jobs))(*jobs)
            L.check(L.lib().oct_pack_weights_batch(self.dt, len(jobs), arr, _stream()), "oct_pack_weights_batch")
            self._packed.update(news)

    def _conv(self, src: Src, wpacked, cout, taps, n, h, w, y0, *, y1=None, split=0, in_mode=L.IN_PLAIN,
              out_mode=L.OUT_PLAIN, bias=None, stats=None, kh=0, kw=0, depth=0, oimg=(0, 0)):
        d = L.ConvDesc(self.dt, n, h, w, src.c0, src.c1, cout, taps,
                       _xf(src.bn0), _xf(src.bn1),
                       in_mode, out_mode, split, 1 if stats is not None else 0, kh, kw, depth, oimg[0], oimg[1])
        a = L.ConvArgs(L.ptr(src.x0), L.ptr(src.x1),
                       L.ptr(src.bn0.scale) if src.bn0 else None, L.ptr(src.bn0.shift) if src.bn0 else None,
                       L.ptr(src.bn1.scale) if src.bn1 else None, L.ptr(src.bn1.shift) if src.bn1 else None,
                       L.ptr(wpacked), L.ptr(bias), L.ptr(y0), L.ptr(y1), L.ptr(stats))
        ev = self._prof_begin()
        L.check(L.lib().oct_conv_forward(C.byref(d), C.byref(a), _stream()), "oct_conv_forward")
        self._prof_end(ev, "igemm", (taps, src.channels, cout, n, h, w, in_mode, out_mode))

    def _stat_blocks(self, cout, n, h, w, src: Src, taps=9, kh=0, kw=0, depth=0):
        d = L.ConvDesc(self.dt, n, h, w, src.c0, src.c1, cout, taps,
                       _xf(src.bn0), _xf(src.bn1), 0, 0, 0, 1, kh, kw, depth, 0, 0)
        return L.lib().oct_conv_stat_blocks(C.byref(d))

    def _wgrad(self, src: Src, dy, cout, taps, n, h, w, dy_mode=L.IN_PLAIN, dbias=None, fused_apply=None, kh=0, kw=0,
               depth=0, in_shift=0, dy_img=(0, 0), dwp=None, partials_ok=True):
        ktot = src.channels
        parts = 1 if (self.deterministic and partials_ok and dwp is None and depth == 0) else 0
        d = L.WgradDesc(self.dt, n, h, w, src.c0, src.c1, cout, taps,
                        _xf(src.bn0), _xf(src.bn1), dy_mode, kh, kw, depth, in_shift,
                        dy_img[0], dy_img[1], parts)
        bias_parts = None
        if parts:
            nparts = L.lib().oct_conv_wgrad_partials(C.byref(d))
            dwp = torch.empty((nparts, taps, cout, ktot), dtype=torch.float32, device=dy.device)
            dwp._oct_nparts = nparts
            if dbias is not None:
                bias_parts = torch.empty((nparts, cout), dtype=torch.float32, device=dy.device)
        elif dwp is None:
            dwp = self._dwp_take(taps * cout * ktot, dy.device).view(taps, cout, ktot)
        a = L.WgradArgs(L.ptr(src.x0), L.ptr(src.x1),
                        L.ptr(src.bn0.scale) if src.bn0 else None, L.ptr(src.bn0.shift) if src.bn0 else None,
                        L.ptr(src.bn1.scale) if src.bn1 else None, L.ptr(src.bn1.shift) if src.bn1 else None,
                        L.ptr(dy), L.ptr(dwp), L.ptr(dbias), *([L.ptr(t) for t in fused_apply] if fused_apply
                                                                 else [None, None, None, None]), L.ptr(bias_parts))
        ev = self._prof_begin()
        L.check(L.lib().oct_conv_wgrad(C.byref(d), C.byref(a), _stream()), "oct_conv_wgrad")
        self._prof_end(ev, "wgrad", (taps, ktot, cout, n, h, w, dy_mode, 0))
        if bias_parts is not None:
            L.check(L.lib().oct_reduce_bias_partials(bias_parts.data_ptr(), nparts, cout,
                                                     cout // 4 if dy_mode == L.IN_S2D else cout, dbias.data_ptr(), 1,
                                                     _stream()), "oct_reduce_bias_partials")
        return dwp

    def _dwp_take(self, numel: int, dev) -> torch.Tensor:
        if self._arena_on:
            lo = self._arena_off
            self._arena_off = lo + (numel + 63) // 64 * 64
            if self._arena is not None and self._arena_off <= self._arena.numel() and self._arena.device == dev:
                return self._arena[lo:lo + numel]
            self._arena_short = True
        return torch.zeros(numel, dtype=torch.float32, device=dev)

    def _arena_begin(self, dev):
        self._arena_on, self._arena_off, self._arena_short = True, 0, False
        self._unpack_jobs = []
        if self._arena is not None and self._arena.device == dev:
            self._arena.zero_()

    def _flush_unpack(self):
        if self._unpack_jobs:
            arr = (L.UnpackJob * len(self._unpack_jobs))(*[j[0] for j in self._unpack_jobs])
            L.check(L.lib().oct_unpack_wgrad_batch(len(self._unpack_jobs), arr, _stream()), "oct_unpack_wgrad_batch")
            self._unpack_jobs = []

    def _arena_end(self, dev):
        self._flush_unpack()
        if self._arena_short or self._arena is None:
            self._arena = torch.empty(self._arena_off, dtype=torch.float32, device=dev)
        self._arena_on = False

    def _unpack(self, mode, dwp, grad, cout, cin, accumulate):
        job = L.UnpackJob(mode, cout, cin, int(accumulate), getattr(dwp, "_oct_nparts", 1), 0, dwp.data_ptr(), grad.data_ptr())
        if self._arena_on:
            self._unpack_jobs.append((job, dwp, grad))
            return
        arr = (L.UnpackJob * 1)(job)
        L.check(L.lib().oct_unpack_wgrad_batch(1, arr, _stream()), "oct_unpack_wgrad_batch")

    def _conv_bn(self, P, keys: ConvKeys, src: Src, cout, n, h, w, train: bool) -> ConvRec:
        wkey, nk = keys.w, keys.bn
        wt = P[wkey]
        dev = wt.device
        cbias = L.ptr(P[keys.b]) if keys.b else None
        wp = self._pack(wkey, wt, L.PACK_CONV_FPROP, cout, src.channels)
        y = self._act(n, h, w, cout, dev)
        scale = torch.empty(cout, dtype=torch.float32, device=dev)
        shift = torch.empty_like(scale)
        if train:
            nblk = self._stat_blocks(cout, n, h, w, src)
            partials = torch.empty((nblk, 2, cout), dtype=torch.float32, device=dev)
            self._conv(src, wp, cout, 9, n, h, w, y, stats=partials)
            mean = torch.empty_like(scale)
            invstd = torch.empty_like(scale)
            L.check(L.lib().oct_bn_finalize(
                partials.data_ptr(), nblk, cout, float(n * h * w), P[nk + ".weight"].data_ptr(),
                P[nk + ".bias"].data_ptr(), BN_EPS, BN_MOMENTUM, P[nk + ".running_mean"].data_ptr(),
                P[nk + ".running_var"].data_ptr(), mean.data_ptr(), invstd.data_ptr(), scale.data_ptr(),
                shift.data_ptr(), cbias, _stream()), "oct_bn_finalize")
            self._nbt.append(P[nk + ".num_batches_tracked"])
            bn = BNState(scale, shift, mean, invstd)
        else:
            self._conv(src, wp, cout, 9, n, h, w, y)
            L.check(L.lib().oct_bn_eval_coeffs(
                cout, P[nk + ".weight"].data_ptr(), P[nk + ".bias"].data_ptr(),
                P[nk + ".running_mean"].data_ptr(), P[nk + ".running_var"].data_ptr(), BN_EPS,
                scale.data_ptr(), shift.data_ptr(), cbias, _stream()), "oct_bn_eval_coeffs")
            if self._frozen_bwd:
                invstd = torch.rsqrt(P[nk + ".running_var"] + BN_EPS)
                mean = P[nk + ".running_mean"] - P[keys.b] if keys.b else P[nk + ".running_mean"]
                bn = BNState(scale, shift, mean, invstd, frozen=True)
            else:
                bn = BNState(scale, shift)
        return ConvRec(wkey, nk + ".weight", nk + ".bias", keys.b, src, y, bn, cout, n, h, w)

    def _block(self, P, blk: BlockSpec, src, n, h, w, train, ctx):
        r1 = self._conv_bn(P, blk.c1, src, blk.cout, n, h, w, train)
        r2 = self._conv_bn(P, blk.c2, Src(r1.y, blk.cout, r1.bn), blk.cout, n, h, w, train)
        ctx.convs[blk.name] = [r1, r2]
        return r2

    def forward(self, P: dict, x: torch.Tensor, train: bool, target: torch.Tensor | None = None,
                loss_cfg=(1.0, 0.0, 1e-7), want_probs=True, want_argmax=False, want_logits=False, defer_loss=False,
                frozen_bwd=False):
        lib = L.lib()
        if x.dim() != 4 or x.shape[1] != self.cin:
            raise RuntimeError(f"expected input (B,{self.cin},H,W), got {tuple(x.shape)}")
        n, _, h, w = x.shape
        sp = self.spec
        if h % sp.divisor or w % sp.divisor:
            raise RuntimeError(
                f"Sizes of tensors must match except in dimension 1. Input {h}x{w} is not divisible by {sp.divisor} "
                f"({len(sp.enc) - 1} 2x2 poolings followed by as many 2x up-samplings)")
        dev = x.device
        if dev.type != "cuda":
            raise L.OctError("the HIP path needs a device tensor (there is no CPU fallback)")
        xf = x.detach().to(torch.float32).contiguous()
        if train or frozen_bwd:
            self._prepack(P)
        self._frozen_bwd = bool(frozen_bwd) and not train
        ctx = Ctx(n=n, h=h, w=w, loss_cfg=tuple(loss_cfg))
        self._nbt = []
        xt = self._act(n, h, w, self.cin, dev)
        L.check(lib.oct_nchw_to_nhwc(self.dt, xf.data_ptr(), xt.data_ptr(), n, self.cin, h, w, _stream()),
                "oct_nchw_to_nhwc")
        src = Src(xt, self.cin)
        hh, ww = h, w
        skips = []
        prev = None
        for li, blk in enumerate(sp.enc):
            prev = self._block(P, blk, src, n, hh, ww, train, ctx)
            if li == len(sp.enc) - 1:
                break
            skips.append(prev)
            pooled = self._act(n, hh // 2, ww // 2, blk.cout, dev)
            L.check(lib.oct_bn_relu_pool_fwd(self.dt, prev.y.data_ptr(), prev.bn.scale.data_ptr(),
                                             prev.bn.shift.data_ptr(), pooled.data_ptr(), n, hh, ww, blk.cout,
                                             _stream()), "oct_bn_relu_pool_fwd")
            hh //= 2
            ww //= 2
            src = Src(pooled, blk.cout)
        for di, ((wkey, bkey, cout_d), blk) in enumerate(zip(sp.ups, sp.dec)):
            cin_d = prev.cout
            wp = self._pack(wkey, P[wkey], L.PACK_DECONV_FPROP, cout_d, cin_d)
            u = self._act(n, hh * 2, ww * 2, cout_d, dev)
            self._conv(Src(prev.y, cin_d, prev.bn), wp, 4 * cout_d, 1, n, hh, ww, u, out_mode=L.OUT_D2S, bias=P[bkey])
            ctx.ups[di] = (prev, u)
            hh *= 2
            ww *= 2
            sk = skips[len(skips) - 1 - di]
            src = (Src(u, cout_d, None, sk.y, sk.cout, sk.bn) if sp.dec_first
                   else Src(sk.y, sk.cout, sk.bn, u, cout_d, None))
            prev = self._block(P, blk, src, n, hh, ww, train, ctx)
        ctx.head_in = prev
        if self._nbt:
            torch._foreach_add_(self._nbt, 1)
            self._nbt = []
        self._frozen_bwd = False
        hd = L.HeadDesc(self.dt, n, h, w, self.f, self.ncls)
        probs = torch.empty((n, self.ncls, h, w), dtype=torch.float32, device=dev) if want_probs else None
        amax = torch.empty((n, h, w), dtype=torch.int64, device=dev) if want_argmax else None
        logits = torch.empty((n, self.ncls, h, w), dtype=torch.float32, device=dev) if want_logits else None
        partials = None
        if target is not None:
            if target.shape != (n, h, w):
                raise RuntimeError(f"target must be (B,H,W)={n, h, w}, got {tuple(target.shape)}")
            target = target.to(device=dev, dtype=torch.int64).contiguous()
            nb = lib.oct_head_blocks(C.byref(hd))
            partials = torch.empty((nb, L.HEAD_LOSS_SLOTS), dtype=torch.float64, device=dev)
            if (defer_loss and loss_cfg[1] == 0.0 and self.f == 32 and self.ncls <= 8
                    and not (want_probs or want_argmax or want_logits)):
                ctx.target = target
                ctx.loss = torch.empty(3, dtype=torch.float32, device=dev)
                ctx.dice_coef = torch.zeros(2 * L.MAX_CLASSES, dtype=torch.float32, device=dev)
                ctx.loss_partials = partials
                return ctx, None, None, None
        L.check(lib.oct_head_forward(C.byref(hd), prev.y.data_ptr(), prev.bn.scale.data_ptr(),
                                     prev.bn.shift.data_ptr(), P[sp.head_w].data_ptr(),
                                     P[sp.head_b].data_ptr(), L.ptr(target), L.ptr(probs), L.ptr(amax),
                                     L.ptr(logits), L.ptr(partials), _stream()), "oct_head_forward")
        if target is not None:
            w_ce, w_dice, eps = loss_cfg
            ctx.target = target
            ctx.loss = torch.empty(3, dtype=torch.float32, device=dev)
            ctx.dice_coef = torch.zeros(2 * L.MAX_CLASSES, dtype=torch.float32, device=dev)
            L.check(lib.oct_head_loss_finalize(C.byref(hd), partials.data_ptr(), partials.shape[0], w_ce, w_dice,
                                               eps, ctx.loss.data_ptr(), ctx.dice_coef.data_ptr(), _stream()),
                    "oct_head_loss_finalize")
        return ctx, probs, amax, logits

    def _bn_backward(self, rec: ConvRec, da, dpool, G, accumulate, partials=None, defer_apply=False):
        lib = L.lib()
        n, h, w, c = rec.n, rec.h, rec.w, rec.cout
        dev = rec.y.device
        pooled = dpool is not None
        g = da if da is not None else self._act(n, h, w, c, dev)
        pool_fused = pooled and partials is None and self.debug is None and bool(lib.oct_bn_bwd_apply_pool_ok(self.dt, n, h, w, c))
        if partials is not None:
            nblk = partials.shape[0]
        else:
            nblk = lib.oct_dact_bn_reduce_blocks(n, h, w, c, 1 if pooled else 0)
            partials = torch.empty((nblk, 2, c), dtype=torch.float32, device=dev)
            L.check(lib.oct_dact_bn_reduce(self.dt, L.ptr(da), L.ptr(dpool), rec.y.data_ptr(), rec.bn.scale.data_ptr(),
                                           rec.bn.shift.data_ptr(), rec.bn.mean.data_ptr(), rec.bn.invstd.data_ptr(),
                                           g.data_ptr() if (pooled and not pool_fused) else None, partials.data_ptr(),
                                           n, h, w, c, _stream()),
                    "oct_dact_bn_reduce")
        coef = torch.empty((3, c), dtype=torch.float32, device=dev)
        L.check(lib.oct_bn_bwd_finalize(partials.data_ptr(), nblk, c, float(n * h * w), self._P[rec.gkey].data_ptr(),
                                        rec.bn.mean.data_ptr(), rec.bn.invstd.data_ptr(), G[rec.gkey].data_ptr(),
                                        G[rec.bkey].data_ptr(), coef.data_ptr(), int(accumulate), _stream()),
                "oct_bn_bwd_finalize")
        if self.debug is not None:
            self.debug["g:" + rec.wkey] = g.float().clone()
        if rec.bn.frozen:
            coef[1:].zero_()
            if rec.cbkey:
                gb = coef[0] * partials[:, 0, :].sum(0)
                G[rec.cbkey].add_(gb) if accumulate else G[rec.cbkey].copy_(gb)
        if defer_apply and not pooled:
            return g, coef
        if pool_fused:
            L.check(lib.oct_bn_bwd_apply_pool(self.dt, L.ptr(da), dpool.data_ptr(), rec.y.data_ptr(), rec.bn.scale.data_ptr(),
                                              rec.bn.shift.data_ptr(), coef.data_ptr(), g.data_ptr(), n, h, w, c, _stream()),
                    "oct_bn_bwd_apply_pool")
            return g
        L.check(lib.oct_bn_bwd_apply(self.dt, g.data_ptr(), rec.y.data_ptr(), coef.data_ptr(),
                                     None if pooled else rec.bn.scale.data_ptr(),
                                     None if pooled else rec.bn.shift.data_ptr(), n * h * w, c, _stream()),
                "oct_bn_bwd_apply")
        if self.debug is not None:
            self.debug["dy:" + rec.wkey] = g.float().clone()
            self.debug["y:" + rec.wkey] = rec.y.float().clone()
            self.debug["coef:" + rec.wkey] = coef.clone()
        return g

    def _conv_backward(self, rec: ConvRec, dy, G, accumulate, need_dx=True):
        n, h, w = rec.n, rec.h, rec.w
        src = rec.src
        cin = src.channels
        dwp = self._wgrad(src, dy, rec.cout, 9, n, h, w)
        self._unpack(L.PACK_CONV_FPROP, dwp, G[rec.wkey], rec.cout, cin, accumulate)
        if not need_dx:
            return None, None
        wp = self._pack(rec.wkey, self._P[rec.wkey], L.PACK_CONV_DGRAD, rec.cout, cin)
        d0 = self._act(n, h, w, src.c0, dy.device)
        d1 = self._act(n, h, w, src.c1, dy.device) if src.c1 else None
        self._conv(Src(dy, rec.cout), wp, cin, 9, n, h, w, d0, y1=d1, split=src.c0 if src.c1 else 0)
        if self.debug is not None:
            def bnc(b):
                return None if b is None else (b.scale.clone(), b.shift.clone())
            self.debug["layer:" + rec.wkey] = dict(
                x0=src.x0.float().clone(), bn0=bnc(src.bn0), x1=None if src.x1 is None else src.x1.float().clone(),
                bn1=bnc(src.bn1), dy=dy.float().clone(), d0=d0.float().clone(), d1=None if d1 is None else d1.float().clone(),
                y=rec.y.float().clone())
        return d0, d1

    def _conv_backward_fused(self, r1: ConvRec, r2: ConvRec, dy2, G, accumulate):
        src = r2.src
        if self.fused_bwd_off or self.debug is not None or self.deterministic or src.c1 or src.bn0 is None or src.bn0 is not r1.bn or src.x0 is not r1.y:
            return None
        lib = L.lib()
        n, h, w, cin, cout = r2.n, r2.h, r2.w, src.c0, r2.cout
        d = L.WgradDesc(self.dt, n, h, w, cin, 0, cout, 9, _xf(src.bn0), L.XF_NONE, L.IN_PLAIN, 0, 0, 0, 0, 0, 0, 0)
        if not lib.oct_conv_backward_fused_ok(C.byref(d)):
            return None
        dev = dy2.device
        wp = self._pack(r2.wkey, self._P[r2.wkey], L.PACK_CONV_DGRAD, cout, cin)
        da1 = self._act(n, h, w, cin, dev)
        dwp = self._dwp_take(9 * cout * cin, dev).view(9, cout, cin)
        parts = torch.empty((lib.oct_conv_backward_fused_blocks(C.byref(d)), 2, cin), dtype=torch.float32, device=dev)
        a = L.ConvBwdFusedArgs(L.ptr(r1.y), L.ptr(r1.bn.scale), L.ptr(r1.bn.shift), L.ptr(r1.bn.mean), L.ptr(r1.bn.invstd),
                               L.ptr(dy2), L.ptr(wp), L.ptr(da1), L.ptr(dwp), L.ptr(parts))
        ev = self._prof_begin()
        L.check(lib.oct_conv_backward_fused(C.byref(d), C.byref(a), _stream()), "oct_conv_backward_fused")
        self._prof_end(ev, "igemm", (9, cout, cin, n, h, w, L.IN_PLAIN, L.OUT_PLAIN))
        self._unpack(L.PACK_CONV_FPROP, dwp, G[r2.wkey], cout, cin, accumulate)
        return da1, parts

    def _block_backward(self, name, da, dpool, G, accumulate, need_dx=True, partials=None):
        r1, r2 = self._ctx.convs[name]
        for r in (r1, r2):
            if r.cbkey and not accumulate and not r.bn.frozen:
                G[r.cbkey].zero_()
        dy2 = self._bn_backward(r2, da, dpool, G, accumulate, partials=partials)
        fused = self._conv_backward_fused(r1, r2, dy2, G, accumulate)
        if fused is not None:
            da1, parts1 = fused
        else:
            (da1, _), parts1 = self._conv_backward(r2, dy2, G, accumulate), None
        first_fused = False
        if not need_dx and r1.src.c1 == 0 and r1.src.bn0 is None:
            qd = L.WgradDesc(self.dt, r1.n, r1.h, r1.w, r1.src.c0, 0, r1.cout, 9, L.XF_NONE, L.XF_NONE, L.IN_PLAIN)
            first_fused = bool(L.lib().oct_conv_wgrad_fused_apply_ok(C.byref(qd)))
        if first_fused:
            da1, coef = self._bn_backward(r1, da1, None, G, accumulate, partials=parts1, defer_apply=True)
            dwp = self._wgrad(r1.src, da1, r1.cout, 9, r1.n, r1.h, r1.w,
                              fused_apply=(r1.y, coef, r1.bn.scale, r1.bn.shift))
            self._unpack(L.PACK_CONV_FPROP, dwp, G[r1.wkey], r1.cout, 1, accumulate)
            return None, None
        dy1 = self._bn_backward(r1, da1, None, G, accumulate, partials=parts1)
        return self._conv_backward(r1, dy1, G, accumulate, need_dx=need_dx)

    def backward_stages(self):
        sp = self.spec

        def blk_keys(b: BlockSpec):
            ks = []
            for c in (b.c1, b.c2):
                ks += [c.w, c.bn + ".weight", c.bn + ".bias"] + ([c.b] if c.b else [])
            return ks
        nd = len(sp.dec)
        stages = []
        for di in range(nd - 1, -1, -1):
            ks = ([sp.head_w, sp.head_b] if di == nd - 1 else []) + blk_keys(sp.dec[di]) + list(sp.ups[di][:2])
            stages.append((f"dec{di}", ks))
        for li in range(len(sp.enc) - 1, -1, -1):
            stages.append((f"enc{li}", blk_keys(sp.enc[li])))
        return stages

    def _stage_done(self, hook, idx):
        if hook is not None and idx in hook.flush_stages:
            self._flush_unpack()
            hook.stage_done(idx)

    def backward(self, P: dict, ctx: Ctx, G: dict, dprobs: torch.Tensor | None = None, accumulate=False,
                 dlogits: torch.Tensor | None = None, stage_hook=None):
        lib = L.lib()
        sp = self.spec
        self._P, self._ctx = P, ctx
        n, h, w, f, ncls = ctx.n, ctx.h, ctx.w, self.f, self.ncls
        rec = ctx.head_in
        dev = rec.y.device
        self._arena_begin(dev)
        hd = L.HeadDesc(self.dt, n, h, w, f, ncls)
        if dprobs is not None:
            dprobs = dprobs.to(torch.float32).contiguous()
            tgt, dc, w_ce = None, None, 0.0
        elif dlogits is None:
            if ctx.target is None:
                raise RuntimeError("backward without an output gradient needs forward(target=...)")
            tgt, dc, w_ce = ctx.target, ctx.dice_coef, ctx.loss_cfg[0]
        hsrc = Src(rec.y, f, rec.bn)
        head_partials = None
        hw, hb = P[sp.head_w], P[sp.head_b]
        bgrad, wgrad_t = G[sp.head_b], G[sp.head_w]
        fused_dw = False
        dl = None
        if f == 32 and dlogits is None:
            fused_dw = ncls <= 8
            if not accumulate:
                bgrad.zero_()
                if fused_dw:
                    wgrad_t.zero_()
            if not fused_dw:
                dl = self._act(n, h, w, ncls, dev)
            da = self._act(n, h, w, f, dev)
            nb = lib.oct_head_blocks(C.byref(hd))
            head_partials = torch.empty((nb, 2, f), dtype=torch.float32, device=dev)
            L.check(lib.oct_head_backward_fused(
                C.byref(hd), rec.y.data_ptr(), rec.bn.scale.data_ptr(), rec.bn.shift.data_ptr(),
                rec.bn.mean.data_ptr(), rec.bn.invstd.data_ptr(), hw.data_ptr(),
                hb.data_ptr(), L.ptr(tgt), L.ptr(dc), w_ce, L.ptr(dprobs), L.ptr(dl), da.data_ptr(),
                head_partials.data_ptr(), bgrad.data_ptr(), wgrad_t.data_ptr() if fused_dw else None,
                L.ptr(ctx.loss_partials) if dprobs is None else None, _stream()),
                "oct_head_backward_fused")
            if ctx.loss_partials is not None and dprobs is None:
                w_ce_, w_dice_, eps_ = ctx.loss_cfg
                L.check(lib.oct_head_loss_finalize(C.byref(hd), ctx.loss_partials.data_ptr(), ctx.loss_partials.shape[0],
                                                   w_ce_, w_dice_, eps_, ctx.loss.data_ptr(), ctx.dice_coef.data_ptr(),
                                                   _stream()), "oct_head_loss_finalize")
        else:
            dl = self._act(n, h, w, ncls, dev)
            if dlogits is not None:
                dlf = dlogits.to(torch.float32).contiguous()
                L.check(lib.oct_nchw_to_nhwc(self.dt, dlf.data_ptr(), dl.data_ptr(), n, ncls, h, w, _stream()),
                        "oct_nchw_to_nhwc")
            else:
                L.check(lib.oct_head_dlogits(C.byref(hd), rec.y.data_ptr(), rec.bn.scale.data_ptr(),
                                             rec.bn.shift.data_ptr(), hw.data_ptr(), hb.data_ptr(), L.ptr(tgt),
                                             L.ptr(dc), w_ce, L.ptr(dprobs), dl.data_ptr(), _stream()),
                        "oct_head_dlogits")
            L.check(lib.oct_channel_sum(self.dt, dl.data_ptr(), bgrad.data_ptr(), n * h * w, ncls, int(accumulate),
                                        _stream()), "oct_channel_sum")
            wp = self._pack(sp.head_w, hw, L.PACK_1X1_DGRAD, ncls, f)
            da = self._act(n, h, w, f, dev)
            self._conv(Src(dl, ncls), wp, f, 1, n, h, w, da)
        if not fused_dw:
            dwp = self._wgrad(hsrc, dl, ncls, 1, n, h, w)
            self._unpack(L.PACK_1X1_FPROP, dwp, wgrad_t, ncls, f, accumulate)
        nd = len(sp.dec)
        dskip = [None] * nd
        for di in range(nd - 1, -1, -1):
            d0, d1 = self._block_backward(sp.dec[di].name, da, None, G, accumulate,
                                          partials=head_partials if di == nd - 1 else None)
            du, dskip[di] = (d0, d1) if sp.dec_first else (d1, d0)
            wkey, bkey, cout_d = sp.ups[di]
            prev, u = ctx.ups[di]
            cin_d = prev.cout
            hl, wl = prev.h, prev.w
            bgrad = G[bkey]
            if not accumulate:
                bgrad.zero_()
            dwp = self._wgrad(Src(prev.y, cin_d, prev.bn), du, 4 * cout_d, 1, n, hl, wl, dy_mode=L.IN_S2D,
                              dbias=bgrad)
            self._unpack(L.PACK_DECONV_FPROP, dwp, G[wkey], cout_d, cin_d, accumulate)
            wp = self._pack(wkey, P[wkey], L.PACK_DECONV_DGRAD, cout_d, cin_d)
            da = self._act(n, hl, wl, cin_d, dev)
            self._conv(Src(du, cout_d), wp, cin_d, 1, n, hl, wl, da, in_mode=L.IN_S2D)
            if self.debug is not None:
                self.debug["up:" + wkey] = dict(x=prev.y.float().clone(), bn=(prev.bn.scale.clone(), prev.bn.shift.clone()),
                                                u=u.float().clone(), du=du.float().clone(), da=da.float().clone(), bkey=bkey)
            self._stage_done(stage_hook, nd - 1 - di)
        dpool, _ = self._block_backward(sp.enc[-1].name, da, None, G, accumulate)
        self._stage_done(stage_hook, nd)
        for li in range(len(sp.enc) - 2, -1, -1):
            dpool, _ = self._block_backward(sp.enc[li].name, dskip[nd - 1 - li], dpool, G, accumulate,
                                            need_dx=(li != 0))
            if li:
                self._stage_done(stage_hook, nd + len(sp.enc) - 1 - li)
        self._arena_end(dev)
        self._stage_done(stage_hook, nd + len(sp.enc) - 1)
        self._P = self._ctx = None
        return G
```

### retinal_oct_image_segmentation_via_deep_learning_amd/engine3d.py

```python
from __future__ import annotations

import ctypes as C

import torch

from . import _lib as L
from .engine import (BN_EPS, BN_MOMENTUM, BNState, BlockSpec, ConvKeys, ConvRec, Ctx, NetSpec, Src, UNetEngine, _stream,
                     ynet_unet_spec)


class UNet3DEngine(UNetEngine):
    def __init__(self, in_channels: int, out_channels: int, features: int = 32, dtype: str = "bf16"):
        super().__init__(in_channels, out_channels, features, dtype, spec=ynet_unet_spec(in_channels, out_channels, features))
        self.supports_frozen_bwd = False

    def _conv_bn3(self, P, keys: ConvKeys, src: Src, cout, n, h, w, depth, train) -> ConvRec:
        wkey, nk = keys.w, keys.bn
        dev = P[wkey].device
        wp = self._pack(wkey, P[wkey], L.PACK_CONV3D_FPROP, cout, src.channels)
        y = self._act(n, h, w, cout, dev)
        scale = torch.empty(cout, dtype=torch.float32, device=dev)
        shift = torch.empty_like(scale)
        if train:
            nblk = self._stat_blocks(cout, n, h, w, src, depth=depth)
            partials = torch.empty((nblk, 2, cout), dtype=torch.float32, device=dev)
            self._conv(src, wp, cout, 9, n, h, w, y, stats=partials, depth=depth)
            mean, invstd = torch.empty_like(scale), torch.empty_like(scale)
            L.check(L.lib().oct_bn_finalize(
                partials.data_ptr(), nblk, cout, float(n * h * w), P[nk + ".weight"].data_ptr(),
                P[nk + ".bias"].data_ptr(), BN_EPS, BN_MOMENTUM, P[nk + ".running_mean"].data_ptr(),
                P[nk + ".running_var"].data_ptr(), mean.data_ptr(), invstd.data_ptr(), scale.data_ptr(),
                shift.data_ptr(), None, _stream()), "oct_bn_finalize")
            self._nbt.append(P[nk + ".num_batches_tracked"])
            bn = BNState(scale, shift, mean, invstd)
        else:
            self._conv(src, wp, cout, 9, n, h, w, y, depth=depth)
            L.check(L.lib().oct_bn_eval_coeffs(
                cout, P[nk + ".weight"].data_ptr(), P[nk + ".bias"].data_ptr(), P[nk + ".running_mean"].data_ptr(),
                P[nk + ".running_var"].data_ptr(), BN_EPS, scale.data_ptr(), shift.data_ptr(), None, _stream()),
                "oct_bn_eval_coeffs")
            bn = BNState(scale, shift)
        rec = ConvRec(wkey, nk + ".weight", nk + ".bias", None, src, y, bn, cout, n, h, w)
        rec.depth = depth
        return rec

    def _block3(self, P, blk: BlockSpec, src, n, h, w, depth, train, ctx):
        r1 = self._conv_bn3(P, blk.c1, src, blk.cout, n, h, w, depth, train)
        r2 = self._conv_bn3(P, blk.c2, Src(r1.y, blk.cout, r1.bn), blk.cout, n, h, w, depth, train)
        ctx.convs[blk.name] = [r1, r2]
        return r2

    def forward(self, P: dict, x: torch.Tensor, train: bool, target: torch.Tensor | None = None,
                loss_cfg=(1.0, 0.0, 1e-7), want_probs=True, want_argmax=False, want_logits=False, defer_loss=False):
        lib = L.lib()
        if x.dim() != 5 or x.shape[1] != self.cin:
            raise RuntimeError(f"expected input (B,{self.cin},D,H,W), got {tuple(x.shape)}")
        b, _, dd, h, w = x.shape
        sp = self.spec
        if dd % sp.divisor or h % sp.divisor or w % sp.divisor:
            raise RuntimeError(f"Sizes of tensors must match except in dimension 1. Volume {dd}x{h}x{w} is not divisible by "
                               f"{sp.divisor} ({len(sp.enc) - 1} 2x2x2 poolings followed by as many 2x up-samplings)")
        dev = x.device
        if dev.type != "cuda":
            raise L.OctError("the HIP path needs a device tensor (there is no CPU fallback)")
        xf = x.detach().to(torch.float32).contiguous()
        ctx = Ctx(n=b, h=dd * h, w=w, loss_cfg=tuple(loss_cfg))
        ctx.vol = (b, dd, h, w)
        ctx.pool2 = {}
        self._nbt = []
        n = b * dd
        xt = self._act(n, h, w, self.cin, dev)
        L.check(lib.oct_nchw_to_nhwc(self.dt, xf.data_ptr(), xt.data_ptr(), b, self.cin, dd * h, w, _stream()), "oct_nchw_to_nhwc")
        src = Src(xt, self.cin)
        hh, ww, dl = h, w, dd
        skips = []
        prev = None
        for li, blk in enumerate(sp.enc):
            prev = self._block3(P, blk, src, b * dl, hh, ww, dl, train, ctx)
            if li == len(sp.enc) - 1:
                break
            skips.append(prev)
            p2 = self._act(b * dl, hh // 2, ww // 2, blk.cout, dev)
            L.check(lib.oct_bn_relu_pool_fwd(self.dt, prev.y.data_ptr(), prev.bn.scale.data_ptr(), prev.bn.shift.data_ptr(),
                                             p2.data_ptr(), b * dl, hh, ww, blk.cout, _stream()), "oct_bn_relu_pool_fwd")
            pooled = self._act(b * dl // 2, hh // 2, ww // 2, blk.cout, dev)
            L.check(lib.oct_depth_pool_fwd(self.dt, p2.data_ptr(), pooled.data_ptr(), b * dl // 2,
                                           (hh // 2) * (ww // 2) * blk.cout, _stream()), "oct_depth_pool_fwd")
            ctx.pool2[blk.name] = p2
            hh //= 2
            ww //= 2
            dl //= 2
            src = Src(pooled, blk.cout)
        for di, ((wkey, bkey, cout_d), blk) in enumerate(zip(sp.ups, sp.dec)):
            cin_d = prev.cout
            u = self._act(2 * b * dl, hh * 2, ww * 2, cout_d, dev)
            for kdi in (0, 1):
                wp = self._pack(f"{wkey}#{kdi}", P[wkey], L.PACK_DECONV3D_FPROP, cout_d, cin_d, kdi)
                self._conv(Src(prev.y, cin_d, prev.bn), wp, 4 * cout_d, 1, b * dl, hh, ww, u, out_mode=L.OUT_D2S,
                           bias=P[bkey], oimg=(2, kdi))
            ctx.ups[di] = (prev, u)
            hh *= 2
            ww *= 2
            dl *= 2
            sk = skips[len(skips) - 1 - di]
            src = Src(u, cout_d, None, sk.y, sk.cout, sk.bn)
            prev = self._block3(P, blk, src, b * dl, hh, ww, dl, train, ctx)
        ctx.head_in = prev
        if self._nbt:
            torch._foreach_add_(self._nbt, 1)
            self._nbt = []
        hd = L.HeadDesc(self.dt, b, dd * h, w, self.f, self.ncls)
        probs = torch.empty((b, self.ncls, dd, h, w), dtype=torch.float32, device=dev) if want_probs else None
        amax = torch.empty((b, dd, h, w), dtype=torch.int64, device=dev) if want_argmax else None
        logits = torch.empty((b, self.ncls, dd, h, w), dtype=torch.float32, device=dev) if want_logits else None
        partials = None
        if target is not None:
            if target.shape != (b, dd, h, w):
                raise RuntimeError(f"target must be (B,D,H,W)={b, dd, h, w}, got {tuple(target.shape)}")
            target = target.to(device=dev, dtype=torch.int64).contiguous()
            nb = lib.oct_head_blocks(C.byref(hd))
            partials = torch.empty((nb, L.HEAD_LOSS_SLOTS), dtype=torch.float64, device=dev)
            if (defer_loss and loss_cfg[1] == 0.0 and self.f == 32 and self.ncls <= 8
                    and not (want_probs or want_argmax or want_logits)):
                ctx.target = target
                ctx.loss = torch.empty(3, dtype=torch.float32, device=dev)
                ctx.dice_coef = torch.zeros(2 * L.MAX_CLASSES, dtype=torch.float32, device=dev)
                ctx.loss_partials = partials
                return ctx, None, None, None
        L.check(lib.oct_head_forward(C.byref(hd), prev.y.data_ptr(), prev.bn.scale.data_ptr(), prev.bn.shift.data_ptr(),
                                     P[sp.head_w].data_ptr(), P[sp.head_b].data_ptr(), L.ptr(target), L.ptr(probs),
                                     L.ptr(amax), L.ptr(logits), L.ptr(partials), _stream()), "oct_head_forward")
        if target is not None:
            w_ce, w_dice, eps = loss_cfg
            ctx.target = target
            ctx.loss = torch.empty(3, dtype=torch.float32, device=dev)
            ctx.dice_coef = torch.zeros(2 * L.MAX_CLASSES, dtype=torch.float32, device=dev)
            L.check(lib.oct_head_loss_finalize(C.byref(hd), partials.data_ptr(), partials.shape[0], w_ce, w_dice, eps,
                                               ctx.loss.data_ptr(), ctx.dice_coef.data_ptr(), _stream()),
                    "oct_head_loss_finalize")
        return ctx, probs, amax, logits

    def _conv_backward(self, rec: ConvRec, dy, G, accumulate, need_dx=True):
        n, h, w, depth = rec.n, rec.h, rec.w, rec.depth
        src = rec.src
        cin = src.channels
        slab = self._dwp_take(27 * rec.cout * cin, dy.device).view(3, 9, rec.cout, cin)
        qd = L.WgradDesc(self.dt, n, h, w, src.c0, src.c1, rec.cout, 9, 0, 0, L.IN_PLAIN, 0, 0, depth, L.IMG_SHIFT_ALL, 0, 0, 0)
        if src.bn0 is None and src.c1 == 0 and not self.deterministic and L.lib().oct_conv_wgrad_all_depth_taps_ok(C.byref(qd)):
            self._wgrad(src, dy, rec.cout, 9, n, h, w, depth=depth, in_shift=L.IMG_SHIFT_ALL, dwp=slab)
        else:
            for kdi in range(3):
                self._wgrad(src, dy, rec.cout, 9, n, h, w, depth=depth, in_shift=kdi - 1, dwp=slab[kdi])
        L.check(L.lib().oct_unpack_wgrad3d(L.PACK_CONV3D_FPROP, slab.data_ptr(), G[rec.wkey].data_ptr(), rec.cout, cin, 0,
                                           int(accumulate), _stream()), "oct_unpack_wgrad3d")
        if not need_dx:
            return None, None
        wp = self._pack(rec.wkey, self._P[rec.wkey], L.PACK_CONV3D_DGRAD, rec.cout, cin)
        d0 = self._act(n, h, w, src.c0, dy.device)
        d1 = self._act(n, h, w, src.c1, dy.device) if src.c1 else None
        self._conv(Src(dy, rec.cout), wp, cin, 9, n, h, w, d0, y1=d1, split=src.c0 if src.c1 else 0, depth=depth)
        return d0, d1

    def _block_backward(self, name, da, dpool, G, accumulate, need_dx=True, partials=None):
        r1, r2 = self._ctx.convs[name]
        dy2 = self._bn_backward(r2, da, dpool, G, accumulate, partials=partials)
        da1, _ = self._conv_backward(r2, dy2, G, accumulate)
        dy1 = self._bn_backward(r1, da1, None, G, accumulate)
        return self._conv_backward(r1, dy1, G, accumulate, need_dx=need_dx)

    def backward(self, P: dict, ctx: Ctx, G: dict, dprobs: torch.Tensor | None = None, accumulate=False,
                 dlogits: torch.Tensor | None = None, stage_hook=None):
        lib = L.lib()
        sp = self.spec
        self._P, self._ctx = P, ctx
        b, dd, h, w = ctx.vol
        f, ncls = self.f, self.ncls
        rec = ctx.head_in
        dev = rec.y.device
        self._arena_begin(dev)
        hd = L.HeadDesc(self.dt, b, dd * h, w, f, ncls)
        nimg = b * dd
        if dprobs is not None:
            dprobs = dprobs.to(torch.float32).contiguous()
            tgt, dc, w_ce = None, None, 0.0
        else:
            if ctx.target is None:
                raise RuntimeError("backward without an output gradient needs forward(target=...)")
            tgt, dc, w_ce = ctx.target, ctx.dice_coef, ctx.loss_cfg[0]
        hw_, hb = P[sp.head_w], P[sp.head_b]
        bgrad, wgrad_t = G[sp.head_b], G[sp.head_w]
        head_partials = None
        if f == 32 and ncls <= 8:
            if not accumulate:
                bgrad.zero_()
                wgrad_t.zero_()
            da = self._act(nimg, h, w, f, dev)
            nb = lib.oct_head_blocks(C.byref(hd))
            head_partials = torch.empty((nb, 2, f), dtype=torch.float32, device=dev)
            L.check(lib.oct_head_backward_fused(
                C.byref(hd), rec.y.data_ptr(), rec.bn.scale.data_ptr(), rec.bn.shift.data_ptr(), rec.bn.mean.data_ptr(),
                rec.bn.invstd.data_ptr(), hw_.data_ptr(), hb.data_ptr(), L.ptr(tgt), L.ptr(dc), w_ce, L.ptr(dprobs), None,
                da.data_ptr(), head_partials.data_ptr(), bgrad.data_ptr(), wgrad_t.data_ptr(),
                L.ptr(ctx.loss_partials) if dprobs is None else None, _stream()), "oct_head_backward_fused")
            if ctx.loss_partials is not None and dprobs is None:
                w_ce_, w_dice_, eps_ = ctx.loss_cfg
                L.check(lib.oct_head_loss_finalize(C.byref(hd), ctx.loss_partials.data_ptr(), ctx.loss_partials.shape[0],
                                                   w_ce_, w_dice_, eps_, ctx.loss.data_ptr(), ctx.dice_coef.data_ptr(),
                                                   _stream()), "oct_head_loss_finalize")
        else:
            dl = self._act(nimg, h, w, ncls, dev)
            L.check(lib.oct_head_dlogits(C.byref(hd), rec.y.data_ptr(), rec.bn.scale.data_ptr(), rec.bn.shift.data_ptr(),
                                         hw_.data_ptr(), hb.data_ptr(), L.ptr(tgt), L.ptr(dc), w_ce, L.ptr(dprobs),
                                         dl.data_ptr(), _stream()), "oct_head_dlogits")
            L.check(lib.oct_channel_sum(self.dt, dl.data_ptr(), bgrad.data_ptr(), nimg * h * w, ncls, int(accumulate), _stream()),
                    "oct_channel_sum")
            wp = self._pack(sp.head_w, hw_, L.PACK_1X1_DGRAD, ncls, f)
            da = self._act(nimg, h, w, f, dev)
            self._conv(Src(dl, ncls), wp, f, 1, nimg, h, w, da)
            dwp = self._wgrad(Src(rec.y, f, rec.bn), dl, ncls, 1, nimg, h, w)
            self._unpack(L.PACK_1X1_FPROP, dwp, wgrad_t, ncls, f, accumulate)
        nd = len(sp.dec)
        dskip = [None] * nd
        for di in range(nd - 1, -1, -1):
            du, dskip[di] = self._block_backward(sp.dec[di].name, da, None, G, accumulate,
                                                 partials=head_partials if di == nd - 1 else None)
            wkey, bkey, cout_d = sp.ups[di]
            prev, _ = ctx.ups[di]
            cin_d, nl, hl, wl = prev.cout, prev.n, prev.h, prev.w
            bg = G[bkey]
            if not accumulate:
                bg.zero_()
            for kdi in (0, 1):
                dwp = self._wgrad(Src(prev.y, cin_d, prev.bn), du, 4 * cout_d, 1, nl, hl, wl, dy_mode=L.IN_S2D, dbias=bg,
                                  dy_img=(2, kdi), partials_ok=False)
                L.check(lib.oct_unpack_wgrad3d(L.PACK_DECONV3D_FPROP, dwp.data_ptr(), G[wkey].data_ptr(), cout_d, cin_d, kdi,
                                               int(accumulate), _stream()), "oct_unpack_wgrad3d")
            wp = self._pack(wkey, P[wkey], L.PACK_DECONV3D_DGRAD, cout_d, cin_d)
            da = self._act(nl, hl, wl, cin_d, dev)
            self._conv(Src(du, cout_d), wp, cin_d, 1, nl, hl, wl, da, in_mode=L.IN_S2D, depth=prev.depth)
            self._stage_done(stage_hook, nd - 1 - di)
        dpool, _ = self._block_backward(sp.enc[-1].name, da, None, G, accumulate)
        self._stage_done(stage_hook, nd)
        for li in range(len(sp.enc) - 2, -1, -1):
            blk = sp.enc[li]
            p2 = ctx.pool2[blk.name]
            dp2 = torch.empty_like(p2)
            L.check(lib.oct_depth_pool_bwd(self.dt, p2.data_ptr(), dpool.data_ptr(), dp2.data_ptr(), p2.shape[0] // 2,
                                           p2.shape[1] * p2.shape[2] * p2.shape[3], _stream()), "oct_depth_pool_bwd")
            dpool, _ = self._block_backward(blk.name, dskip[nd - 1 - li], dp2, G, accumulate, need_dx=(li != 0))
            if li:
                self._stage_done(stage_hook, nd + len(sp.enc) - 1 - li)
        self._arena_end(dev)
        self._stage_done(stage_hook, nd + len(sp.enc) - 1)
        self._P = self._ctx = None
        return G
```

Before: 1240 B-scans/s.

## Split head backward into sums and apply passes to avoid materializing da

```diff
diff --git a/include/oct_hip.h b/include/oct_hip.h
--- a/include/oct_hip.h
+++ b/include/oct_hip.h
@@ -206,6 +206,17 @@
                             const float* dprobs, void* dlogits, void* da, float* partials,
                             float* dbias, float* dweight, double* loss_partials, void* stream);
 
+int oct_head_backward_two_pass_ok(const OctHeadDesc* d, int has_target, int has_dprobs, int wants_dlogits);
+int oct_head_backward_sums(const OctHeadDesc* d, const void* y, const float* scale, const float* shift,
+                           const float* mean, const float* invstd, const float* w, const float* b,
+                           const int64_t* target, const float* dice_coef, float w_ce,
+                           const float* dprobs, void* dlogits, float* partials, float* dbias,
+                           float* dweight, double* loss_partials, void* stream);
+int oct_head_backward_apply(const OctHeadDesc* d, const void* y, const float* scale, const float* shift,
+                            const float* w, const float* b, const int64_t* target,
+                            const float* dice_coef, float w_ce, const float* dprobs, void* dlogits,
+                            const float* coef, void* dy, void* stream);
+
 #define OCT_SEG_NHWC 0
 #define OCT_SEG_NCHW 1
 int oct_seg_loss_blocks(size_t npix, int classes);
diff --git a/retinal_oct_image_segmentation_via_deep_learning_amd/_lib.py b/retinal_oct_image_segmentation_via_deep_learning_amd/_lib.py
--- a/retinal_oct_image_segmentation_via_deep_learning_amd/_lib.py
+++ b/retinal_oct_image_segmentation_via_deep_learning_amd/_lib.py
@@ -154,6 +154,12 @@
     "oct_head_backward_fused": (c_int, [C.POINTER(HeadDesc), c_void_p, c_void_p, c_void_p, c_void_p, c_void_p, c_void_p,
                                         c_void_p, c_void_p, c_void_p, c_float, c_void_p, c_void_p, c_void_p, c_void_p,
                                         c_void_p, c_void_p, c_void_p, c_void_p]),
+    "oct_head_backward_two_pass_ok": (c_int, [C.POINTER(HeadDesc), c_int, c_int, c_int]),
+    "oct_head_backward_sums": (c_int, [C.POINTER(HeadDesc), c_void_p, c_void_p, c_void_p, c_void_p, c_void_p, c_void_p,
+                                       c_void_p, c_void_p, c_void_p, c_float, c_void_p, c_void_p, c_void_p, c_void_p,
+                                       c_void_p, c_void_p, c_void_p]),
+    "oct_head_backward_apply": (c_int, [C.POINTER(HeadDesc), c_void_p, c_void_p, c_void_p, c_void_p, c_void_p, c_void_p,
+                                        c_void_p, c_float, c_void_p, c_void_p, c_void_p, c_void_p, c_void_p]),
     "oct_seg_loss_blocks": (c_int, [c_size_t, c_int]),
     "oct_seg_loss_forward": (c_int, [C.POINTER(HeadDesc), c_int, c_void_p, c_void_p, c_void_p, c_void_p, c_void_p]),
     "oct_seg_loss_backward": (c_int, [C.POINTER(HeadDesc), c_int, c_void_p, c_void_p, c_void_p, c_float, c_void_p, c_void_p,
diff --git a/retinal_oct_image_segmentation_via_deep_learning_amd/csrc/head.hip b/retinal_oct_image_segmentation_via_deep_learning_amd/csrc/head.hip
--- a/retinal_oct_image_segmentation_via_deep_learning_amd/csrc/head.hip
+++ b/retinal_oct_image_segmentation_via_deep_learning_amd/csrc/head.hip
@@ -3,10 +3,10 @@
 #include <stdlib.h>
 
 #define HEAD_THREADS 256
-int oct_head_backward_mfma(const OctHeadDesc* d, const void* y, const float* scale, const float* shift, const float* mean,
-                           const float* invstd, const float* w, const float* b, const int64_t* target,
-                           const float* dice_coef, float w_ce, void* da, float* partials, float* dbias, float* dweight,
-                           double* loss_partials, int grid, void* stream);
+int oct_head_backward_mfma(int mode, const OctHeadDesc* d, const void* y, const float* scale, const float* shift,
+                           const float* mean, const float* invstd, const float* w, const float* b, const int64_t* target,
+                           const float* dice_coef, float w_ce, const float* coef, void* out, float* partials, float* dbias,
+                           float* dweight, double* loss_partials, int grid, void* stream);
 #define HEAD_MAX_FEAT 128
 
 struct HeadParams {
@@ -488,6 +488,15 @@
   return oct_check_launch("head_dlogits");
 }
 
+static bool head_mfma_on() {
+  static int on = -1;
+  if (on < 0) { const char* e = getenv("OCT_HEAD_MFMA"); on = (e && e[0] == '0') ? 0 : 1; }
+  return on != 0;
+}
+static bool head_mfma_shape_ok(const OctHeadDesc* d) {
+  return d->dtype == OCT_DT_BF16 && d->feat == 32 && d->classes <= 8;
+}
+
 extern "C" int oct_head_backward_fused(const OctHeadDesc* d, const void* y, const float* scale, const float* shift,
                                        const float* mean, const float* invstd, const float* w, const float* b,
                                        const int64_t* target, const float* dice_coef, float w_ce, const float* dprobs,
@@ -506,11 +515,9 @@
   OCT_CHECK(dlogits || dweight, "oct_head_backward_fused: without dlogits the weight gradient must be fused (dweight)");
   OCT_CHECK(!loss_partials || target, "oct_head_backward_fused: loss partials need a target");
   {
-    static int mfma_on = -1;
-    if (mfma_on < 0) { const char* e = getenv("OCT_HEAD_MFMA"); mfma_on = (e && e[0] == '0') ? 0 : 1; }
-    if (mfma_on && d->dtype == OCT_DT_BF16 && d->classes <= 8 && target && !dprobs && dweight && !dlogits)
-      return oct_head_backward_mfma(d, y, scale, shift, mean, invstd, w, b, target, dice_coef, w_ce, da, partials, dbias,
-                                    dweight, loss_partials, head_grid(d), stream);
+    if (head_mfma_on() && head_mfma_shape_ok(d) && target && !dprobs && dweight && !dlogits)
+      return oct_head_backward_mfma(0, d, y, scale, shift, mean, invstd, w, b, target, dice_coef, w_ce, nullptr, da, partials,
+                                    dbias, dweight, loss_partials, head_grid(d), stream);
   }
   const int grid = head_grid(d);
   hipStream_t s = as_stream(stream);
@@ -528,3 +535,38 @@
 #undef LAUNCH
   return oct_check_launch("head_bwd_fused");
 }
+
+extern "C" int oct_head_backward_two_pass_ok(const OctHeadDesc* d, int has_target, int has_dprobs, int wants_dlogits) {
+  static int on = -1;
+  if (on < 0) { const char* e = getenv("OCT_HEAD_TWO_PASS"); on = (e && e[0] == '0') ? 0 : 1; }
+  if (!d || !on || !head_mfma_on()) return 0;
+  if (d->n <= 0 || d->h <= 0 || d->w <= 0 || d->classes <= 0) return 0;
+  return head_mfma_shape_ok(d) && has_target && !has_dprobs && !wants_dlogits ? 1 : 0;
+}
+
+extern "C" int oct_head_backward_sums(const OctHeadDesc* d, const void* y, const float* scale, const float* shift,
+                                      const float* mean, const float* invstd, const float* w, const float* b,
+                                      const int64_t* target, const float* dice_coef, float w_ce, const float* dprobs,
+                                      void* dlogits, float* partials, float* dbias, float* dweight,
+                                      double* loss_partials, void* stream) {
+  int rc = head_check(d, "oct_head_backward_sums");
+  if (rc) return rc;
+  OCT_CHECK(oct_head_backward_two_pass_ok(d, target != nullptr, dprobs != nullptr, dlogits != nullptr),
+            "oct_head_backward_sums: not eligible (oct_head_backward_two_pass_ok): bf16, feat 32, classes <= 8, labels, no dprobs, no dlogits");
+  OCT_CHECK(y && scale && shift && mean && invstd && w && b && partials && dbias && dweight, "oct_head_backward_sums: null pointer");
+  return oct_head_backward_mfma(1, d, y, scale, shift, mean, invstd, w, b, target, dice_coef, w_ce, nullptr, nullptr, partials,
+                                dbias, dweight, loss_partials, head_grid(d), stream);
+}
+
+extern "C" int oct_head_backward_apply(const OctHeadDesc* d, const void* y, const float* scale, const float* shift,
+                                       const float* w, const float* b, const int64_t* target, const float* dice_coef,
+                                       float w_ce, const float* dprobs, void* dlogits, const float* coef, void* dy,
+                                       void* stream) {
+  int rc = head_check(d, "oct_head_backward_apply");
+  if (rc) return rc;
+  OCT_CHECK(oct_head_backward_two_pass_ok(d, target != nullptr, dprobs != nullptr, dlogits != nullptr),
+            "oct_head_backward_apply: not eligible (oct_head_backward_two_pass_ok): bf16, feat 32, classes <= 8, labels, no dprobs, no dlogits");
+  OCT_CHECK(y && scale && shift && w && b && coef && dy, "oct_head_backward_apply: null pointer");
+  return oct_head_backward_mfma(2, d, y, scale, shift, nullptr, nullptr, w, b, target, dice_coef, w_ce, coef, dy, nullptr,
+                                nullptr, nullptr, nullptr, head_grid(d), stream);
+}
diff --git a/retinal_oct_image_segmentation_via_deep_learning_amd/csrc/head_mfma.hip b/retinal_oct_image_segmentation_via_deep_learning_amd/csrc/head_mfma.hip
--- a/retinal_oct_image_segmentation_via_deep_learning_amd/csrc/head_mfma.hip
+++ b/retinal_oct_image_segmentation_via_deep_learning_amd/csrc/head_mfma.hip
@@ -6,6 +6,7 @@
   const bf16_t* y; const float* scale; const float* shift; const float* mean; const float* invstd;
   const float* w; const float* b; const int64_t* target; const float* dice_coef;
   bf16_t* da; float* partials; float* dbias; float* dweight; double* loss_partials;
+  const float* coef; bf16_t* dy;
   float w_ce; int classes; unsigned npix;
 };
 
@@ -33,10 +34,14 @@
 __device__ __forceinline__ float hm_other(float v) { return __shfl_xor(v, 32); }
 __device__ __forceinline__ unsigned hm_other(unsigned v) { return (unsigned)__shfl_xor((int)v, 32); }
 
+enum { HM_FULL = 0, HM_SUMS = 1, HM_APPLY = 2 };
+
+template <int MODE>
 __global__ void __launch_bounds__(HM_THREADS, 2) head_bwd_mfma_kernel(const HeadMfmaParams p) {
   typedef Mma<bf16_t> M;
   typedef M::Frag Frag;
   constexpr int F = 32;
+  constexpr bool SUMS = MODE != HM_APPLY;
   __shared__ float red[HM_THREADS / 64][2 * F + 8];
   __shared__ float sdw[8 * F];
   __shared__ __attribute__((aligned(16))) unsigned char tiles[HM_THREADS / 64][2][32 * 64];
@@ -45,8 +50,10 @@
   const int tid = threadIdx.x, lane = tid & 63, wave = tid >> 6;
   const int r = lane & 31, hh = lane >> 5;
   const int ncls = p.classes;
-  for (int i = tid; i < 8 * F; i += HM_THREADS) sdw[i] = 0.f;
-  for (int i = tid; i < (int)sizeof(tiles) / 4; i += HM_THREADS) reinterpret_cast<unsigned*>(&tiles[0][0][0])[i] = 0u;
+  if constexpr (SUMS) {
+    for (int i = tid; i < 8 * F; i += HM_THREADS) sdw[i] = 0.f;
+    for (int i = tid; i < (int)sizeof(tiles) / 4; i += HM_THREADS) reinterpret_cast<unsigned*>(&tiles[0][0][0])[i] = 0u;
+  }
   if (p.dice_coef) for (int i = tid; i < 2 * OCT_MAX_CLASSES; i += HM_THREADS) sdc[i] = p.dice_coef[i];
   __syncthreads();
 
@@ -77,6 +84,16 @@
   float bias4[4];
 #pragma unroll
   for (int i = 0; i < 4; ++i) bias4[i] = (4 * hh + i) < ncls ? p.b[4 * hh + i] : 0.f;
+  float k0[16], k1[16], k2[16];
+  if constexpr (MODE == HM_APPLY) {
+#pragma unroll
+    for (int q = 0; q < 2; ++q)
+#pragma unroll
+      for (int j = 0; j < 8; ++j) {
+        const int f = 16 * q + 8 * hh + j;
+        k0[8 * q + j] = p.coef[f]; k1[8 * q + j] = p.coef[F + f]; k2[8 * q + j] = p.coef[2 * F + f];
+      }
+  }
 
   float s1[16], s2[16], sdb[4], ce = 0.f;
   f32x16 accw;
@@ -124,7 +141,7 @@
 #pragma unroll
     for (int k = 0; k < 16; ++k) {
       const float z = fmaf(yv[k], sc[k], sh[k]);
-      zmask |= z > 0.f ? (1u << k) : 0u;
+      if constexpr (SUMS) zmask |= z > 0.f ? (1u << k) : 0u;
       av[k] = fmaxf(z, 0.f);
     }
 #pragma unroll
@@ -163,7 +180,7 @@
 #pragma unroll
       for (int i = 0; i < 4; ++i) dl[i] = fmaf(pr[i], dp[i] - dot, dl[i]);
     }
-    if (p.loss_partials) {
+    if (SUMS && p.loss_partials) {
       float lt = 0.f;
       bool mine = false;
 #pragma unroll
@@ -176,7 +193,7 @@
 #pragma unroll
     for (int i = 0; i < 4; ++i) {
       dl[i] = (valid && (4 * hh + i) < ncls) ? (float)(bf16_t)dl[i] : 0.f;
-      sdb[i] += dl[i];
+      if constexpr (SUMS) sdb[i] += dl[i];
     }
     dpk[0] = hm_pack(dl[0], dl[1]); dpk[1] = hm_pack(dl[2], dl[3]);
     const unsigned o0 = hm_other(dpk[0]), o1 = hm_other(dpk[1]);
@@ -203,7 +220,22 @@
       dq[0] = rA0; dq[1] = rA1; dq[2] = cpk[2]; dq[3] = cpk[3];
       dq[4] = rB0; dq[5] = rB1; dq[6] = cpk[6]; dq[7] = cpk[7];
     }
-    if (valid) {
+    if constexpr (MODE == HM_APPLY) {
+      unsigned oq[8];
+#pragma unroll
+      for (int j = 0; j < 8; ++j) {
+        const float g0 = av[2 * j] > 0.f ? hm_lo(dq[j]) : 0.f, g1 = av[2 * j + 1] > 0.f ? hm_hi(dq[j]) : 0.f;
+        oq[j] = hm_pack(fmaf(k0[2 * j], g0, fmaf(k1[2 * j], yv[2 * j], k2[2 * j])),
+                        fmaf(k0[2 * j + 1], g1, fmaf(k1[2 * j + 1], yv[2 * j + 1], k2[2 * j + 1])));
+      }
+      if (valid) {
+        const hm_u32x4 o0v = {oq[0], oq[1], oq[2], oq[3]}, o1v = {oq[4], oq[5], oq[6], oq[7]};
+        __builtin_nontemporal_store(o0v, reinterpret_cast<hm_u32x4*>(p.dy + (size_t)pix * F + 8 * hh));
+        __builtin_nontemporal_store(o1v, reinterpret_cast<hm_u32x4*>(p.dy + (size_t)pix * F + 16 + 8 * hh));
+      }
+      continue;
+    }
+    if (MODE == HM_FULL && valid) {
       const hm_u32x4 o0v = {dq[0], dq[1], dq[2], dq[3]}, o1v = {dq[4], dq[5], dq[6], dq[7]};
       *reinterpret_cast<hm_u32x4*>(p.da + (size_t)pix * F + 8 * hh) = o0v;
       *reinterpret_cast<hm_u32x4*>(p.da + (size_t)pix * F + 16 + 8 * hh) = o1v;
@@ -223,6 +255,7 @@
       M::mma(accw, hm_tr_frag(d_tile + k16 * 16 * 64 + tr_off), hm_tr_frag(a_tile + k16 * 16 * 64 + tr_off));
   }
 
+  if constexpr (MODE == HM_APPLY) return;
 #pragma unroll
   for (int k = 0; k < 16; ++k) {
     float a = s1[k], b = s2[k];
@@ -270,15 +303,19 @@
   }
 }
 
-int oct_head_backward_mfma(const OctHeadDesc* d, const void* y, const float* scale, const float* shift, const float* mean,
-                           const float* invstd, const float* w, const float* b, const int64_t* target,
-                           const float* dice_coef, float w_ce, void* da, float* partials, float* dbias, float* dweight,
-                           double* loss_partials, int grid, void* stream) {
+int oct_head_backward_mfma(int mode, const OctHeadDesc* d, const void* y, const float* scale, const float* shift,
+                           const float* mean, const float* invstd, const float* w, const float* b, const int64_t* target,
+                           const float* dice_coef, float w_ce, const float* coef, void* out, float* partials, float* dbias,
+                           float* dweight, double* loss_partials, int grid, void* stream) {
   HeadMfmaParams p;
   p.y = (const bf16_t*)y; p.scale = scale; p.shift = shift; p.mean = mean; p.invstd = invstd; p.w = w; p.b = b;
-  p.target = target; p.dice_coef = dice_coef; p.da = (bf16_t*)da; p.partials = partials; p.dbias = dbias;
-  p.dweight = dweight; p.loss_partials = loss_partials; p.w_ce = w_ce; p.classes = d->classes;
+  p.target = target; p.dice_coef = dice_coef; p.da = mode == HM_FULL ? (bf16_t*)out : nullptr; p.partials = partials;
+  p.dbias = dbias; p.dweight = dweight; p.loss_partials = loss_partials; p.coef = coef;
+  p.dy = mode == HM_APPLY ? (bf16_t*)out : nullptr; p.w_ce = w_ce; p.classes = d->classes;
   p.npix = (unsigned)((size_t)d->n * d->h * d->w);
-  hipLaunchKernelGGL(head_bwd_mfma_kernel, dim3(grid), dim3(HM_THREADS), 0, as_stream(stream), p);
-  return oct_check_launch("head_bwd_mfma");
+  hipStream_t s = as_stream(stream);
+  if (mode == HM_FULL) hipLaunchKernelGGL(head_bwd_mfma_kernel<HM_FULL>, dim3(grid), dim3(HM_THREADS), 0, s, p);
+  else if (mode == HM_SUMS) hipLaunchKernelGGL(head_bwd_mfma_kernel<HM_SUMS>, dim3(grid), dim3(HM_THREADS), 0, s, p);
+  else hipLaunchKernelGGL(head_bwd_mfma_kernel<HM_APPLY>, dim3(grid), dim3(HM_THREADS), 0, s, p);
+  return oct_check_launch(mode == HM_FULL ? "head_bwd_mfma" : mode == HM_SUMS ? "head_bwd_mfma_sums" : "head_bwd_mfma_apply");
 }
diff --git a/retinal_oct_image_segmentation_via_deep_learning_amd/engine.py b/retinal_oct_image_segmentation_via_deep_learning_amd/engine.py
--- a/retinal_oct_image_segmentation_via_deep_learning_amd/engine.py
+++ b/retinal_oct_image_segmentation_via_deep_learning_amd/engine.py
@@ -147,6 +147,7 @@
         self.rowdot_off = os.environ.get("OCT_ROWDOT", "1") == "0"
         self.deterministic = os.environ.get("OCT_DETERMINISTIC", "0") == "1"
         self.fused_bwd_off = False
+        self.head_two_pass_off = False
         self.debug = None
         self.prof = None
         self.prof_labels = None
@@ -439,7 +440,7 @@
                     "oct_head_loss_finalize")
         return ctx, probs, amax, logits
 
-    def _bn_backward(self, rec: ConvRec, da, dpool, G, accumulate, partials=None, defer_apply=False):
+    def _bn_backward(self, rec: ConvRec, da, dpool, G, accumulate, partials=None, defer_apply=False, head_apply=None):
         lib = L.lib()
         n, h, w, c = rec.n, rec.h, rec.w, rec.cout
         dev = rec.y.device
@@ -470,6 +471,9 @@
                 G[rec.cbkey].add_(gb) if accumulate else G[rec.cbkey].copy_(gb)
         if defer_apply and not pooled:
             return g, coef
+        if head_apply is not None:
+            head_apply(coef, g)
+            return g
         if pool_fused:
             L.check(lib.oct_bn_bwd_apply_pool(self.dt, L.ptr(da), dpool.data_ptr(), rec.y.data_ptr(), rec.bn.scale.data_ptr(),
                                               rec.bn.shift.data_ptr(), coef.data_ptr(), g.data_ptr(), n, h, w, c, _stream()),
@@ -528,12 +532,12 @@
         self._unpack(L.PACK_CONV_FPROP, dwp, G[r2.wkey], cout, cin, accumulate)
         return da1, parts
 
-    def _block_backward(self, name, da, dpool, G, accumulate, need_dx=True, partials=None):
+    def _block_backward(self, name, da, dpool, G, accumulate, need_dx=True, partials=None, head_apply=None):
         r1, r2 = self._ctx.convs[name]
         for r in (r1, r2):
             if r.cbkey and not accumulate and not r.bn.frozen:
                 G[r.cbkey].zero_()
-        dy2 = self._bn_backward(r2, da, dpool, G, accumulate, partials=partials)
+        dy2 = self._bn_backward(r2, da, dpool, G, accumulate, partials=partials, head_apply=head_apply)
         fused = self._conv_backward_fused(r1, r2, dy2, G, accumulate)
         if fused is not None:
             da1, parts1 = fused
@@ -551,6 +555,33 @@
             return None, None
         dy1 = self._bn_backward(r1, da1, None, G, accumulate, partials=parts1)
         return self._conv_backward(r1, dy1, G, accumulate, need_dx=need_dx)
+
+    def _head_backward_two_pass(self, hd, rec: ConvRec, hw, hb, tgt, dc, w_ce, bgrad, wgrad_t, accumulate):
+        lib = L.lib()
+        ctx = self._ctx
+        dev = rec.y.device
+        if not accumulate:
+            bgrad.zero_()
+            wgrad_t.zero_()
+        nb = lib.oct_head_blocks(C.byref(hd))
+        partials = torch.empty((nb, 2, hd.feat), dtype=torch.float32, device=dev)
+        L.check(lib.oct_head_backward_sums(
+            C.byref(hd), rec.y.data_ptr(), rec.bn.scale.data_ptr(), rec.bn.shift.data_ptr(), rec.bn.mean.data_ptr(),
+            rec.bn.invstd.data_ptr(), hw.data_ptr(), hb.data_ptr(), L.ptr(tgt), L.ptr(dc), w_ce, None, None,
+            partials.data_ptr(), bgrad.data_ptr(), wgrad_t.data_ptr(), L.ptr(ctx.loss_partials), _stream()),
+            "oct_head_backward_sums")
+        if ctx.loss_partials is not None:
+            w_ce_, w_dice_, eps_ = ctx.loss_cfg
+            scratch = torch.empty_like(ctx.dice_coef)
+            L.check(lib.oct_head_loss_finalize(C.byref(hd), ctx.loss_partials.data_ptr(), ctx.loss_partials.shape[0],
+                                               w_ce_, w_dice_, eps_, ctx.loss.data_ptr(), scratch.data_ptr(), _stream()),
+                    "oct_head_loss_finalize")
+
+        def head_apply(coef, dy):
+            L.check(lib.oct_head_backward_apply(
+                C.byref(hd), rec.y.data_ptr(), rec.bn.scale.data_ptr(), rec.bn.shift.data_ptr(), hw.data_ptr(), hb.data_ptr(),
+                L.ptr(tgt), L.ptr(dc), w_ce, None, None, coef.data_ptr(), dy.data_ptr(), _stream()), "oct_head_backward_apply")
+        return None, partials, head_apply
 
     def backward_stages(self):
         sp = self.spec
@@ -597,7 +628,13 @@
         bgrad, wgrad_t = G[sp.head_b], G[sp.head_w]
         fused_dw = False
         dl = None
-        if f == 32 and dlogits is None:
+        head_apply = None
+        two_pass = (dlogits is None and not self.head_two_pass_off and self.debug is None and
+                    bool(lib.oct_head_backward_two_pass_ok(C.byref(hd), int(tgt is not None), int(dprobs is not None), 0)))
+        if two_pass:
+            da, head_partials, head_apply = self._head_backward_two_pass(hd, rec, hw, hb, tgt, dc, w_ce, bgrad, wgrad_t, accumulate)
+            fused_dw = True
+        elif f == 32 and dlogits is None:
             fused_dw = ncls <= 8
             if not accumulate:
                 bgrad.zero_()
@@ -643,7 +680,8 @@
         dskip = [None] * nd
         for di in range(nd - 1, -1, -1):
             d0, d1 = self._block_backward(sp.dec[di].name, da, None, G, accumulate,
-                                          partials=head_partials if di == nd - 1 else None)
+                                          partials=head_partials if di == nd - 1 else None,
+                                          head_apply=head_apply if di == nd - 1 else None)
             du, dskip[di] = (d0, d1) if sp.dec_first else (d1, d0)
             wkey, bkey, cout_d = sp.ups[di]
             prev, u = ctx.ups[di]
diff --git a/retinal_oct_image_segmentation_via_deep_learning_amd/engine3d.py b/retinal_oct_image_segmentation_via_deep_learning_amd/engine3d.py
--- a/retinal_oct_image_segmentation_via_deep_learning_amd/engine3d.py
+++ b/retinal_oct_image_segmentation_via_deep_learning_amd/engine3d.py
@@ -161,9 +161,9 @@
         self._conv(Src(dy, rec.cout), wp, cin, 9, n, h, w, d0, y1=d1, split=src.c0 if src.c1 else 0, depth=depth)
         return d0, d1
 
-    def _block_backward(self, name, da, dpool, G, accumulate, need_dx=True, partials=None):
+    def _block_backward(self, name, da, dpool, G, accumulate, need_dx=True, partials=None, head_apply=None):
         r1, r2 = self._ctx.convs[name]
-        dy2 = self._bn_backward(r2, da, dpool, G, accumulate, partials=partials)
+        dy2 = self._bn_backward(r2, da, dpool, G, accumulate, partials=partials, head_apply=head_apply)
         da1, _ = self._conv_backward(r2, dy2, G, accumulate)
         dy1 = self._bn_backward(r1, da1, None, G, accumulate)
         return self._conv_backward(r1, dy1, G, accumulate, need_dx=need_dx)
@@ -190,7 +190,11 @@
         hw_, hb = P[sp.head_w], P[sp.head_b]
         bgrad, wgrad_t = G[sp.head_b], G[sp.head_w]
         head_partials = None
-        if f == 32 and ncls <= 8:
+        head_apply = None
+        if (not self.head_two_pass_off and self.debug is None and
+                lib.oct_head_backward_two_pass_ok(C.byref(hd), int(tgt is not None), int(dprobs is not None), 0)):
+            da, head_partials, head_apply = self._head_backward_two_pass(hd, rec, hw_, hb, tgt, dc, w_ce, bgrad, wgrad_t, accumulate)
+        elif f == 32 and ncls <= 8:
             if not accumulate:
                 bgrad.zero_()
                 wgrad_t.zero_()
@@ -223,7 +227,8 @@
         dskip = [None] * nd
         for di in range(nd - 1, -1, -1):
             du, dskip[di] = self._block_backward(sp.dec[di].name, da, None, G, accumulate,
-                                                 partials=head_partials if di == nd - 1 else None)
+                                                 partials=head_partials if di == nd - 1 else None,
+                                                 head_apply=head_apply if di == nd - 1 else None)
             wkey, bkey, cout_d = sp.ups[di]
             prev, _ = ctx.ups[di]
             cin_d, nl, hl, wl = prev.cout, prev.n, prev.h, prev.w
```

Measured after the change: 1246 B-scans/s (median of 6 runs). No clear change (+0.4%).
